# Mahdi-Si/VAE-TEB

Measured on AMD Instinct MI355X. Metric: train samples/sec + ELBO, 4096-pt windows, batch 256, 1/2/4/8 MI355X, higher is better.
Workload: dtype bf16 MFMA (decoder heads + conv blocks + ResidualMLP linears, LSTM recurrences f16 fwd / bf16 bwd), fp32 accumulation; fp32 LayerNorm / BatchNorm / LSTM state / front-end / optimizer

## Files before the change

### include/vaeteb.h

```cpp
#ifndef VAETEB_H
#define VAETEB_H

#include <stdint.h>

#ifdef __cplusplus
extern "C" {
#endif

#define VT_OK 0
#define VT_ERR_ARG (-1)
#define VT_ERR_LAYOUT (-2)
#define VT_ERR_HIP (-3)

#define VT_FFT_MAX_LDS 8192

const char* vt_last_error(void);
int vt_stream_fork(void* from, void* to);
int vt_stream_mark(void* stream, int* slot);
int vt_stream_wait_mark(void* stream, int slot);
int vt_abi_version(void);
int vt_arrive_reset(void* stream);
int vt_capture_info(void* stream, char* buf, int len);
int vt_set_h16_format(int fp16);
int vt_get_h16_format(void);
// ... 153 lines not shown
int vt_resmlp_bf16_fwd(int n_layers, const int* dims, const int* layer_ln, const int* layer_act, int skip, float eps,
                       const float* const* params, const float* x, int64_t rows, float* out, float* xhat, float* rstd,
                       void* stream);
int vt_resmlp_bf16_bwd(int n_layers, const int* dims, const int* layer_ln, const int* layer_act, int skip, float eps,
                       const float* const* params, const float* dout, const float* xhat, const float* rstd,
                       int64_t rows, float* dx, float* const* grads, int accumulate, float* ws, int64_t ws_floats,
                       void* stream);
int vt_resmlp_bf16_plan(int n_layers, const int* dims, const int* layer_ln, const int* layer_act, int skip, float eps,
                        const float* const* params, int64_t rows, int64_t* handle, void* stream);
int vt_resmlp_bf16_prep_batch(int n, const int64_t* handles, void* stream);
int vt_resmlp_bf16_fwd_prepped(int n_layers, const int* dims, const int* layer_ln, const int* layer_act, int skip,
                               float eps, const float* const* params, const float* x, int64_t rows, float* out,
                               float* xhat, float* rstd, void* stream);
int vt_resmlp_bf16_split_sizes(int n_layers, const int* dims, const int* layer_ln, const int* layer_act, int skip,
                               int64_t rows, int64_t* sizes);
int vt_resmlp_bf16_bwd_data(int n_layers, const int* dims, const int* layer_ln, const int* layer_act, int skip,
                            float eps, const float* const* params, const float* dout, const float* xhat,
                            const float* rstd, int64_t rows, float* dx, float* const* grads, int accumulate,
                            void* dz16, float* ws, int64_t ws_floats, void* stream);
int vt_resmlp_bf16_bwd_weight(int n_layers, const int* dims, const int* layer_ln, const int* layer_act, int skip,
                              float eps, const float* const* params, const float* xhat, const void* dz16,
                              int64_t rows, float* const* grads, int accumulate, float* ws, int64_t ws_floats,
                              void* stream);
int vt_resmlp_bf16_set_stamps(void* buf);

int vt_mfma_supported(int K, int N);
int vt_mfma_workspace_floats(int64_t R, int K, int N, int64_t* floats);
int vt_mfma_weight_shadow(const float* W, int N, int K, void* W16, void* W16t, void* stream);
int vt_mfma_linear_fwd(const float* X, int64_t R, int K, const void* W16, int N, const float* bias, float* Y,
                       float* ws, int64_t ws_floats, void* stream);
int vt_mfma_linear_bwd_data(const float* dY, int64_t R, int N, const void* W16t, int K, float* dX, int accumulate,
                            float* ws, int64_t ws_floats, void* stream);
int vt_mfma_linear_bwd_weight(const float* dY, int64_t R, int N, const float* X, int K, float* dW, float* db,
                              int accumulate, float* ws, int64_t ws_floats, void* stream);

int vt_conv1d_out_len(int L_in, int K, int mode, int up);
int vt_conv1d_fwd(const float* X, int B, int L_in, int Cin, const float* W, int Cout, int K, int mode, int up,
                  float* Y, void* stream);
int vt_conv1d_bwd_data(const float* dY, int B, int L_in, int Cin, const float* W, int Cout, int K, int mode, int up,
                       float* dX, int accumulate, float* gpad, void* stream);
int vt_conv1d_bwd_weight(const float* dY, const float* X, int B, int L_in, int Cin, int Cout, int K, int mode, int up,
                         float* dW, int accumulate, float* ws, int64_t ws_floats, void* stream);
int vt_conv1d_bn_workspace_floats(int B, int L_in, int Cin, int Cout, int K, int mode, int up, int64_t* floats);
int vt_conv1d_bn_fwd(const float* X, int B, int L_in, int Cin, const float* W, int Cout, int K, int mode, int up,
                     const float* gamma, const float* beta, int act, float eps, float momentum, float* conv_out,
                     float* Y, float* mean, float* rstd, float* run_mean, float* run_var, float* ws,
                     int64_t ws_floats, void* stream);
int vt_conv1d_bf16_shadow(const float* W, int Cout, int Cin, int K, void* w16, void* w16t, void* stream);
int vt_conv1d_bf16_shadow_batch(int n, const int64_t* W, const int* Cout, const int* Cin, const int* K,
                                const int64_t* w16, const int64_t* w16t, void* stream);
int vt_conv_bf16_set_staging(int mode);
int vt_conv_bf16_set_kernels(int flags);
int vt_conv1d_bn_fwd_bf16(const float* X, int B, int L_in, int Cin, const void* w16, int Cout, int K, int mode,
                          int up, const float* gamma, const float* beta, int act, float eps, float momentum,
                          float* conv_out, float* Y, float* mean, float* rstd, float* run_mean, float* run_var,
                          float* ws, int64_t ws_floats, void* stream);
int vt_conv1d_bn_fwd_bf16_in(const float* X, const float* in_mean, const float* in_rstd, const float* in_gamma,
                             const float* in_beta, int in_act, int B, int L_in, int Cin, const void* w16, int Cout,
                             int K, int mode, int up, const float* gamma, const float* beta, int act, float eps,
                             float momentum, float* conv_out, float* Y, float* mean, float* rstd, float* run_mean,
                             float* run_var, float* ws, int64_t ws_floats, void* stream);
int vt_conv1d_fwd_bf16(const float* X, int B, int L_in, int Cin, const void* w16, int Cout, int K, int mode, int up,
                       float* Y, void* stream);
int vt_conv1d_bwd_gpad_bf16(const float* dY, int B, int L_in, int Cin, const void* w16t, int Cout, int K, int mode,
                            int up, float* gpad, void* stream);
int vt_conv1d_bwd_weight_bf16(const float* dY, const float* X, int B, int L_in, int Cin, int Cout, int K, int mode,
                              int up, float* dW, int accumulate, float* ws, int64_t ws_floats, void* stream);
int vt_conv1d_bwd_gpad_bf16_bn(const float* dY, const float* Xc, const float* bnp, int act, int64_t M, int B,
                               int L_in, int Cin, const void* w16t, int Cout, int K, int mode, int up, float* gpad,
                               void* dxbn16, void* stream);
int vt_conv1d_bwd_dx_bf16_bn(const float* dY, const float* Xc, const float* bnp, int act, int64_t M, int B, int L_in,
                             int Cin, const void* w16t, int Cout, int K, int mode, int up, float* dX, float* edge,
                             void* dxbn16, void* stream);
int vt_conv1d_bwd_weight_bf16_dy16(const void* dY16, const float* X, int B, int L_in, int Cin, int Cout, int K,
                                   int mode, int up, float* dW, int accumulate, float* ws, int64_t ws_floats,
                                   void* stream);
int vt_conv1d_bwd_weight_bf16_dy16s(const void* dY16, int dys, const float* X, int B, int L_in, int Cin, int Cout,
                                    int K, int mode, int up, float* dW, int accumulate, float* ws, int64_t ws_floats,
                                    void* stream);
int vt_conv1d_bwd_weight_bf16_in(const float* dY, const void* dY16, int dys, const float* X, const float* in_mean,
                                 const float* in_rstd, const float* in_gamma, const float* in_beta, int in_act, int B,
                                 int L_in, int Cin, int Cout, int K, int mode, int up, float* dW, int accumulate,
                                 float* ws, int64_t ws_floats, void* stream);
int vt_batchnorm_bwd_x16(const float* dY, const float* Xc, const float* bnp, int act, int64_t M, int C, void* d16,
                         void* stream);
int vt_conv1d_bwd_dx16(const void* d16, int B, int L_in, int Cin, const void* w16t, int Cout, int K, int mode, int up,
                       float* dX, float* edge, void* stream);
int vt_conv1d_direct_fwd(const float* X, int B, int L_in, int Cin, const float* W, int Cout, int K, int mode, int up,
                         float* Y, void* stream);
int vt_conv1d_direct_bwd_gpad(const float* dY, int B, int L_in, int Cin, const float* W, int Cout, int K, int mode,
                              int up, float* gpad, void* stream);
int vt_conv1d_fold(const float* gpad, int B, int L_in, int Cin, int Cout, int K, int mode, int up, float* dX,
                   int accumulate, void* stream);
int vt_conv1d_direct_bwd_weight(const float* dY, const float* X, int B, int L_in, int Cin, int Cout, int K, int mode,
                                int up, float* dW, int accumulate, float* ws, int64_t ws_floats, void* stream);

int vt_layernorm_fwd(const float* x, int64_t R, int C, const float* gamma, const float* beta, int act, float eps,
                     float* y, float* xhat, float* rstd, void* stream);
int vt_layernorm_bwd(const float* dy, const float* xhat, const float* rstd, int64_t R, int C, const float* gamma,
                     const float* beta, int act, float* dx, float* dgamma, float* dbeta, int accumulate_params,
                     float* ws, int64_t ws_floats, void* stream);
int vt_batchnorm_fwd(const float* x, int64_t M, int C, const float* gamma, const float* beta, int act, float eps,
                     float momentum, float* y, float* mean, float* rstd, float* run_mean, float* run_var, float* ws,
                     int64_t ws_floats, void* stream);
int vt_batchnorm_bwd(const float* dy, const float* x, int64_t M, int C, const float* mean, const float* rstd,
                     const float* gamma, const float* beta, int act, float* dx, float* dgamma, float* dbeta,
                     int accumulate_params, float* ws, int64_t ws_floats, void* stream);
int vt_batchnorm_fwd_dropout(const float* x, int64_t M, int C, const float* gamma, const float* beta, int act,
                             float eps, float momentum, float* y, float* mean, float* rstd, float* run_mean,
                             float* run_var, int L, float p, int64_t seed, const void* seed_offset, float* ws,
                             int64_t ws_floats, void* stream);
int vt_batchnorm_bwd_dropout(const float* dy, const float* x, int64_t M, int C, const float* mean, const float* rstd,
                             const float* gamma, const float* beta, int act, int L, float p, int64_t seed,
                             const void* seed_offset, float* dx, float* dgamma, float* dbeta, int accumulate_params,
                             float* ws, int64_t ws_floats, void* stream);
int vt_batchnorm_bwd_coef(const float* dy, const float* x, int64_t M, int C, const float* mean, const float* rstd,
                          const float* gamma, const float* beta, int act, float* dgamma, float* dbeta,
                          int accumulate_params, float* bnp, float* ws, int64_t ws_floats, void* stream);
int vt_batchnorm_eval(const float* x, int64_t M, int C, const float* run_mean, const float* run_var, float eps,
                      const float* gamma, const float* beta, int act, float* y, void* stream);
int vt_syncbn_sums(const float* x, const float* dy, int64_t M, int C, int which, const float* mean,
                   const float* rstd, const float* gamma, const float* beta, int act, double* sums, float* ws,
                   int64_t ws_floats, void* stream);
int vt_syncbn_stats(const double* sums, int C, int which, float eps, float momentum, float* mean, float* rstd,
                    float* run_mean, float* run_var, float* dgamma, float* dbeta, int accumulate, void* stream);
int vt_batchnorm_apply(const float* x, int64_t M, int C, const float* mean, const float* rstd, const float* gamma,
                       const float* beta, int act, float* y, void* stream);
int vt_syncbn_bwd_dx(const float* dy, const float* x, int64_t M, int C, const float* mean, const float* rstd,
                     const float* gamma, const float* beta, int act, const double* sums, float* dx, float* ws,
                     void* stream);
int vt_act_fwd(const float* x, int64_t n, int act, float* y, void* stream);
int vt_act_bwd(const float* dy, const float* x, int64_t n, int act, float* dx, void* stream);

int vt_lstm_layer_fwd(const float* gin, const float* w_hh, const float* b_hh, int B, int S, int hidden, float* out_h,
                      float* out_hprev, float* out_c, float* gates, void* stream);
int vt_lstm_layer_bwd(const float* dh_out, const float* gates, const float* cst, const float* w_hh, int B, int S,
                      int hidden, float* dgates, void* stream);
int vt_lstm_layer_fwd_x(const float* x, int In, const float* w_ih, const float* b_ih, const float* w_hh,
                        const float* b_hh, int B, int S, int hidden, float* out_h, float* out_hprev, float* out_c,
                        float* gates, void* stream);
int vt_lstm_layer_bwd_x(const float* dh_out, const float* gates, const float* cst, const float* w_hh,
                        const float* w_ih, int In, int B, int S, int hidden, float* dgates, float* dx, void* stream);
int vt_lstm16_layer_fwd(const float* x, int In, const float* w_ih, const float* b_ih, const float* w_hh,
                        const float* b_hh, int B, int S, int hidden, float* out_h, float* out_hprev, float* out_c,
                        float* gates, void* stream);
int vt_lstm16_layer_bwd(const float* dh_out, const float* gates, const float* cst, const float* w_hh,
                        const float* w_ih, int In, int B, int S, int hidden, float* dgates, float* dx, void* stream);
int vt_lstm16_pair_fwd(const float* x, int In, const float* w_ih0, const float* b_ih0, const float* w_hh0,
                       const float* b_hh0, const float* w_ih1, const float* b_ih1, const float* w_hh1,
                       const float* b_hh1, int B, int seq, int hidden, float* h0, float* c0, float* gates0, float* h1,
                       float* c1, float* gates1, void* stream);
int vt_lstm16_pair_bwd(const float* dh_out, const float* gates1, const float* c1, const float* w_hh1,
                       const float* w_ih1, const float* gates0, const float* c0, const float* w_hh0,
                       const float* w_ih0, int In0, int B, int seq, int hidden, void* dgates1, void* dgates0,
                       float* dx, void* stream, int dg_bf16);
int vt_lstm16_quad_fwd(const float* x, int In, const float* const* params, int B, int seq, int hidden,
                       float* const* outs, void* stream);
int vt_lstm16_quad_bwd(const float* dh_out, const float* const* w, const float* const* gc, int In0, int B, int seq,
                       int hidden, void* const* dg, float* dmid, float* dx, void* stream, int dg_bf16);
int vt_lstm16_chain_errors(int* count, int reset);
int vt_lstm_layer_bwd_weight(const float* dgates, const float* x, int In, const float* hprev, int B, int S,
                             int hidden, float* dw_ih, float* dw_hh, float* db_ih, float* db_hh, int accumulate,
                             float* ws, int64_t ws_floats, void* stream);
int vt_lstm16_layer_bwd_weight(const float* dgates, const float* x, int In, const float* h, int B, int S,
                               int hidden, float* dw_ih, float* dw_hh, float* db_ih, float* db_hh, int accumulate,
                               float* ws, int64_t ws_floats, void* stream);
// ... 60 lines not shown
```

### vae-teb_amd/csrc/conv.h

```cpp
#pragma once
#include "bnbwd.h"
#include "common.h"

namespace vt {

struct Geo {
    int B, L_in, Cin, Cout, K, up, mode, L_up, pad, L_out;
};

__device__ __forceinline__ float up_lerp(float a, float b, float l1) {
#pragma clang fp contract(off)
    return (1.f - l1) * a + l1 * b;
}

template <bool IBN = false>
__device__ __forceinline__ float src_val(const float* __restrict__ xb, const Geo& g, int tp, int ci,
                                         const float* ip = nullptr, int cs = 0, int iact = 0) {
    int t = tp - g.pad;
    if (g.mode == 0) {
        if (t < 0 || t >= g.L_up) return 0.f;
    } else if (g.L_up <= g.pad) {
        t = t < 0 ? 0 : (t >= g.L_up ? g.L_up - 1 : t);
    } else {
        t = t < 0 ? -t : t;
        t = t >= g.L_up ? 2 * (g.L_up - 1) - t : t;
    }
    if (!g.up) {
        const float v = xb[(int64_t)t * g.Cin + ci];
        return IBN ? bn_relu_at(ip, cs, ci, v) : v;
    }
    float s = (t + 0.5f) * 0.5f - 0.5f;
    s = s < 0.f ? 0.f : s;
    const int i0 = (int)s;
    const int i1 = i0 + 1 < g.L_in ? i0 + 1 : g.L_in - 1;
    const float l1 = s - (float)i0;
    float a = xb[(int64_t)i0 * g.Cin + ci], b = xb[(int64_t)i1 * g.Cin + ci];
    if constexpr (IBN) {
        a = bn_relu_at(ip, cs, ci, a);
        b = bn_relu_at(ip, cs, ci, b);
    }
    return up_lerp(a, b, l1);
}


__device__ __forceinline__ bool src_row(const Geo& g, int tp, int& i0, int& i1, float& l1) {
    int t = tp - g.pad;
    if (g.mode == 0) {
        if (t < 0 || t >= g.L_up) return false;
    } else if (g.L_up <= g.pad) {
        t = t < 0 ? 0 : (t >= g.L_up ? g.L_up - 1 : t);
    } else {
        t = t < 0 ? -t : t;
        t = t >= g.L_up ? 2 * (g.L_up - 1) - t : t;
    }
    if (!g.up) {
        i0 = i1 = t;
        l1 = 0.f;
        return true;
    }
    float s = (t + 0.5f) * 0.5f - 0.5f;
    s = s < 0.f ? 0.f : s;
    i0 = (int)s;
    i1 = i0 + 1 < g.L_in ? i0 + 1 : g.L_in - 1;
    l1 = s - (float)i0;
    return true;
}

__device__ __forceinline__ void src_span(const Geo& g, int t0, int n, int& lo, int& hi) {
    const int ta = t0 - g.pad, tz = t0 + n - 1 - g.pad;
    int a = 0x7fffffff, z = -1;
    if (g.mode == 0) {
        a = ta > 0 ? ta : 0;
        z = tz < g.L_up - 1 ? tz : g.L_up - 1;
    } else if (g.L_up <= g.pad) {
        a = 0;
        z = g.L_up - 1;
    } else {
        if (tz >= 0 && ta <= g.L_up - 1) {
            a = ta > 0 ? ta : 0;
            z = tz < g.L_up - 1 ? tz : g.L_up - 1;
        }
        if (ta < 0) {
            const int l = -tz > 1 ? -tz : 1;
            a = l < a ? l : a;
            z = -ta > z ? -ta : z;
        }
        if (tz >= g.L_up) {
            const int l = 2 * (g.L_up - 1) - tz;
            const int h = 2 * (g.L_up - 1) - (ta > g.L_up ? ta : g.L_up);
            a = l < a ? l : a;
            z = h > z ? h : z;
        }
    }
    if (z < a) {
        lo = 0;
        hi = -1;
        return;
    }
    if (!g.up) {
        lo = a;
        hi = z;
        return;
    }
    float sa = (a + 0.5f) * 0.5f - 0.5f, sz = (z + 0.5f) * 0.5f - 0.5f;
    sa = sa < 0.f ? 0.f : sa;
    sz = sz < 0.f ? 0.f : sz;
    lo = (int)sa;
    hi = (int)sz + 1 < g.L_in ? (int)sz + 1 : g.L_in - 1;
}

template <int NC, bool IBN = false>
__device__ __forceinline__ void src_vec(const float* __restrict__ xb, const Geo& g, int tp, int cb, bool ok,
                                        float (&v)[NC], const float* ip = nullptr, int cs = 0, int iact = 0) {
    int i0 = 0, i1 = 0;
    float l1 = 0.f;
    const bool in = ok && src_row(g, tp, i0, i1, l1);
    const float* p0 = xb + (int64_t)(in ? i0 : 0) * g.Cin;
    const float* p1 = xb + (int64_t)(in ? i1 : 0) * g.Cin;
    float a[NC], b[NC];
#pragma unroll
    for (int j = 0; j < NC; ++j) {
        const int c = cb + j < g.Cin ? cb + j : g.Cin - 1;
        a[j] = p0[c];
        b[j] = g.up ? p1[c] : 0.f;
    }
    if constexpr (IBN) {
#pragma unroll
        for (int j = 0; j < NC; ++j) {
            a[j] = bn_relu_at(ip, cs, cb + j, a[j]);
            b[j] = g.up ? bn_relu_at(ip, cs, cb + j, b[j]) : 0.f;
        }
    }
#pragma unroll
    for (int j = 0; j < NC; ++j)
        v[j] = (in && cb + j < g.Cin) ? (g.up ? up_lerp(a[j], b[j], l1) : a[j]) : 0.f;
}

static inline Geo geo(int B, int L_in, int Cin, int Cout, int K, int mode, int up) {
    Geo g;
    g.B = B; g.L_in = L_in; g.Cin = Cin; g.Cout = Cout; g.K = K; g.mode = mode; g.up = up;
    g.L_up = L_in * (up ? 2 : 1);
    g.pad = mode == 0 ? K - 1 : (K - 1) / 2;
    g.L_out = mode == 0 ? g.L_up : g.L_up + 2 * g.pad - K + 1;
    return g;
}


static inline int cdiv(int a, int b) { return (a + b - 1) / b; }

int bn_stats_finalize_launch(const float* stats, int tiles_per_sample, int B, int TP, int Lo, int C, float eps,
                             float momentum, float* mean, float* rstd, float* run_mean, float* run_var,
                             hipStream_t st);
int sum_splits_launch(const float* part, int splits, int64_t n, float* out, int accumulate, hipStream_t st,
                      int pK = 0, int pCo = 0, int pCi = 0);
int cfw16_launch(const float* x, const Geo& g, const void* w16, float* y, int Lo, float* stats, hipStream_t st,
                 const BnIn* ibn = nullptr);
void fold_edges_launch(float* dx, const float* edge, int B, int L, int pad, int C, hipStream_t st);
int bn_apply_launch(const float* x, int64_t M, int C, const float* mean, const float* rstd, const float* gamma,
                    const float* beta, int act, float* y, hipStream_t st);

}
```

### vae-teb_amd/csrc/conv_bf16.hip

```cpp
#include <stdlib.h>

#include "conv.h"
#include "h16.h"

namespace vt {

int g_conv_kern = 11;

namespace {

constexpr int CB = 32;
constexpr int RS = 40;

template <int K, int NT>
struct BCfg {
    static constexpr int PM = NT <= 2 ? 4 : 2;
    static constexpr int TC = 16 * NT, TP = 64 * PM, WIN = TP + K - 1;
    static constexpr int XB = WIN * RS, WB = K * TC * RS;
    static constexpr int LDS_BYTES = (XB + WB) * 2 > 8 * TC * 4 ? (XB + WB) * 2 : 8 * TC * 4;
};

struct FoldOut {
    int pad, L;
    float* edge;
// ... 469 lines not shown
        case 10: return bf_k<10>(x, g, w16, cin32, y, Lo, stats, st, bn, fo, ibn);
        default: return bf_k<11>(x, g, w16, cin32, y, Lo, stats, st, bn, fo, ibn);
    }
}

__global__ void k_conv_fold_edges(float* __restrict__ dx, const float* __restrict__ edge, int L, int pad, int C) {
    const int i = blockIdx.x * blockDim.x + threadIdx.x;
    if (i >= 2 * pad * C) return;
    const int r = i / C, c = i - r * C, b = blockIdx.y;
    const int s = r < pad ? 1 + r : L - 1 - pad + (r - pad);
    if (s < 0 || s > L - 1 || (r < pad && s < 1) || (r >= pad && s >= 1 && s <= pad)) return;
    const float* eb = edge + (int64_t)b * 2 * pad * C + c;
    float* o = dx + ((int64_t)b * L + s) * C + c;
    float v = *o;
    if (s >= 1 && s <= pad) v += eb[(pad - s) * C];
    const int tr = pad + 2 * (L - 1) - s;
    if (s <= L - 2 && tr < L + 2 * pad && tr >= pad + L) v += eb[(tr - L) * C];
    *o = v;
}

constexpr int KMAXB = 11;

}

void fold_edges_launch(float* dx, const float* edge, int B, int L, int pad, int C, hipStream_t st) {
    hipLaunchKernelGGL(k_conv_fold_edges, dim3((unsigned)((2 * pad * C + 255) / 256), (unsigned)B), dim3(256), 0, st,
                       dx, edge, L, pad, C);
}
}

using namespace vt;

extern "C" {

int vt_conv_bf16_set_staging(int mode) {
    VT_CHECK_ARG(mode >= 0 && mode <= 2, "vt_conv_bf16_set_staging: mode %d not in 0..2", mode);
    g_conv_cl = mode;
    return VT_OK;
}

int vt_conv_bf16_set_kernels(int flags) {
    VT_CHECK_ARG(flags >= 0 && flags <= 15, "vt_conv_bf16_set_kernels: flags %d not in 0..15", flags);
    g_conv_kern = flags;
    return VT_OK;
}

int vt_conv1d_bf16_shadow(const float* W, int Cout, int Cin, int K, void* w16, void* w16t, void* stream) {
    VT_CHECK_ARG(Cout > 0 && Cin > 0 && K > 0 && K <= KMAXB, "vt_conv1d_bf16_shadow: shape");
    const int cin32 = cdiv(Cin, 32) * 32, cout32 = cdiv(Cout, 32) * 32;
    const int64_t n = (int64_t)Cout * K * cin32 + (int64_t)Cin * K * cout32;
    VT_H16(hipLaunchKernelGGL(k_conv_shadow<H>, dim3((unsigned)((n + 255) / 256)), dim3(256), 0, S(stream), W, Cout,
                              Cin, K, cin32, cout32, (H*)w16, (H*)w16t));
    VT_LAUNCH_CHECK("vt_conv1d_bf16_shadow");
    return VT_OK;
}

int vt_conv1d_bf16_shadow_batch(int n, const int64_t* W, const int* Cout, const int* Cin, const int* K,
                                const int64_t* w16, const int64_t* w16t, void* stream) {
    VT_CHECK_ARG(n >= 0 && n <= CSB_MAX, "vt_conv1d_bf16_shadow_batch: %d weights (at most %d)", n, CSB_MAX);
    if (n == 0) return VT_OK;
    ConvShadowBatch cb{};
    cb.n = n;
    cb.prefix[0] = 0;
    for (int h = 0; h < n; ++h) {
        VT_CHECK_ARG(W[h] && w16[h] && w16t[h] && Cout[h] > 0 && Cin[h] > 0 && K[h] > 0 && K[h] <= KMAXB,
                     "vt_conv1d_bf16_shadow_batch: weight %d", h);
        cb.W[h] = reinterpret_cast<const float*>(W[h]);
        cb.Cout[h] = Cout[h];
        cb.Cin[h] = Cin[h];
        cb.K[h] = K[h];
        cb.w16[h] = reinterpret_cast<void*>(w16[h]);
        cb.w16t[h] = reinterpret_cast<void*>(w16t[h]);
        const int64_t e = (int64_t)Cout[h] * K[h] * (cdiv(Cin[h], 32) * 32) + (int64_t)Cin[h] * K[h] * (cdiv(Cout[h], 32) * 32);
        cb.prefix[h + 1] = cb.prefix[h] + (int)((e + 255) / 256);
    }
    VT_H16(hipLaunchKernelGGL(k_conv_shadow_batch<H>, dim3((unsigned)cb.prefix[n]), dim3(256), 0, S(stream), cb));
    VT_LAUNCH_CHECK("vt_conv1d_bf16_shadow_batch");
    return VT_OK;
}

static int bn_fwd_bf16(const float* X, int B, int L_in, int Cin, const void* w16, int Cout, int K, int mode, int up,
                       const float* gamma, const float* beta, int act, float eps, float momentum, float* conv_out,
                       float* Y, float* mean, float* rstd, float* run_mean, float* run_var, float* ws,
                       int64_t ws_floats, hipStream_t st, const BnIn* ibn, const char* who) {
    VT_CHECK_ARG(B > 0 && L_in > 0 && Cin > 0 && Cout > 0 && K > 0 && K <= KMAXB && (mode == 0 || mode == 1),
                 "%s: shape (K <= %d)", who, KMAXB);
    Geo g = geo(B, L_in, Cin, Cout, K, mode, up);
    const int cin32 = cdiv(Cin, 32) * 32;
    const int TP = bf_launch(nullptr, g, nullptr, cin32, nullptr, g.L_out, nullptr, nullptr);
    const int tps = cdiv(g.L_out, TP);
    VT_CHECK_ARG(ws && ws_floats >= (int64_t)B * tps * 2 * Cout, "%s: workspace too small", who);
    if (bf_launch(X, g, w16, cin32, conv_out, g.L_out, ws, st, nullptr, FoldOut{-1, 0, nullptr}, ibn) < 0) return VT_ERR_ARG;
    bn_stats_finalize_launch(ws, tps, B, TP, g.L_out, Cout, eps, momentum, mean, rstd, run_mean, run_var, st);
    if (Y) bn_apply_launch(conv_out, (int64_t)B * g.L_out, Cout, mean, rstd, gamma, beta, act, Y, st);
    VT_LAUNCH_CHECK(who);
    return VT_OK;
}

int vt_conv1d_bn_fwd_bf16(const float* X, int B, int L_in, int Cin, const void* w16, int Cout, int K, int mode,
                          int up, const float* gamma, const float* beta, int act, float eps, float momentum,
                          float* conv_out, float* Y, float* mean, float* rstd, float* run_mean, float* run_var,
                          float* ws, int64_t ws_floats, void* stream) {
    return bn_fwd_bf16(X, B, L_in, Cin, w16, Cout, K, mode, up, gamma, beta, act, eps, momentum, conv_out, Y, mean,
                       rstd, run_mean, run_var, ws, ws_floats, S(stream), nullptr, "vt_conv1d_bn_fwd_bf16");
}

int vt_conv1d_bn_fwd_bf16_in(const float* X, const float* in_mean, const float* in_rstd, const float* in_gamma,
                             const float* in_beta, int in_act, int B, int L_in, int Cin, const void* w16, int Cout,
                             int K, int mode, int up, const float* gamma, const float* beta, int act, float eps,
                             float momentum, float* conv_out, float* Y, float* mean, float* rstd, float* run_mean,
                             float* run_var, float* ws, int64_t ws_floats, void* stream) {
    VT_CHECK_ARG(in_mean && in_rstd && in_gamma && in_beta && in_act == 1,
                 "vt_conv1d_bn_fwd_bf16_in: input BatchNorm parameters (ReLU blocks only)");
    const BnIn bi{in_mean, in_rstd, in_gamma, in_beta, in_act};
    return bn_fwd_bf16(X, B, L_in, Cin, w16, Cout, K, mode, up, gamma, beta, act, eps, momentum, conv_out, Y, mean,
                       rstd, run_mean, run_var, ws, ws_floats, S(stream), &bi, "vt_conv1d_bn_fwd_bf16_in");
}

int vt_conv1d_fwd_bf16(const float* X, int B, int L_in, int Cin, const void* w16, int Cout, int K, int mode, int up,
                       float* Y, void* stream) {
    VT_CHECK_ARG(B > 0 && L_in > 0 && Cin > 0 && Cout > 0 && K > 0 && K <= KMAXB && (mode == 0 || mode == 1),
                 "vt_conv1d_fwd_bf16: shape (K <= %d)", KMAXB);
    Geo g = geo(B, L_in, Cin, Cout, K, mode, up);
    if (bf_launch(X, g, w16, cdiv(Cin, 32) * 32, Y, g.L_out, nullptr, S(stream)) < 0) return VT_ERR_ARG;
    VT_LAUNCH_CHECK("vt_conv1d_fwd_bf16");
    return VT_OK;
}

static int bwd_gpad(const float* dY, int B, int L_in, int Cin, const void* w16t, int Cout, int K, int mode, int up,
                    float* gpad, hipStream_t st, const BnB* bn, const char* who,
                    FoldOut fo = FoldOut{-1, 0, nullptr}) {
    VT_CHECK_ARG(B > 0 && L_in > 0 && Cin > 0 && Cout > 0 && K > 0 && K <= KMAXB, "%s: shape", who);
    Geo f = geo(B, L_in, Cin, Cout, K, mode, up);
    Geo g = geo(B, f.L_out, Cout, Cin, K, 0, 0);
    if (bf_launch(dY, g, w16t, cdiv(Cout, 32) * 32, gpad, f.L_out + K - 1, nullptr, st, bn, fo) < 0) return VT_ERR_ARG;
    VT_LAUNCH_CHECK(who);
    return VT_OK;
}

int vt_conv1d_bwd_gpad_bf16(const float* dY, int B, int L_in, int Cin, const void* w16t, int Cout, int K, int mode,
                            int up, float* gpad, void* stream) {
    return bwd_gpad(dY, B, L_in, Cin, w16t, Cout, K, mode, up, gpad, S(stream), nullptr, "vt_conv1d_bwd_gpad_bf16");
}

int vt_conv1d_bwd_gpad_bf16_bn(const float* dY, const float* Xc, const float* bnp, int act, int64_t M, int B,
                               int L_in, int Cin, const void* w16t, int Cout, int K, int mode, int up, float* gpad,
                               void* dxbn16, void* stream) {
    VT_CHECK_ARG(Xc && bnp && act >= 0 && act <= 3 && M > 0, "vt_conv1d_bwd_gpad_bf16_bn: BatchNorm arguments");
    const BnB bn{Xc, bnp, act, 1.f / (float)M, dxbn16};
    return bwd_gpad(dY, B, L_in, Cin, w16t, Cout, K, mode, up, gpad, S(stream), &bn, "vt_conv1d_bwd_gpad_bf16_bn");
}

int vt_conv1d_bwd_dx_bf16_bn(const float* dY, const float* Xc, const float* bnp, int act, int64_t M, int B, int L_in,
                             int Cin, const void* w16t, int Cout, int K, int mode, int up, float* dX, float* edge,
                             void* dxbn16, void* stream) {
    VT_CHECK_ARG(Xc && bnp && act >= 0 && act <= 3 && M > 0, "vt_conv1d_bwd_dx_bf16_bn: BatchNorm arguments");
    const Geo f = geo(B, L_in, Cin, Cout, K, mode, up);
    VT_CHECK_ARG(!up && (mode == 0 || f.L_up > f.pad) && (mode == 0 || f.pad == 0 || edge),
                 "vt_conv1d_bwd_dx_bf16_bn: geometry (no upsample, reflect needs L > pad and an edge buffer)");
    const BnB bn{Xc, bnp, act, 1.f / (float)M, dxbn16};
    const FoldOut fo{f.pad, L_in, mode == 0 ? nullptr : edge};
    const int rc = bwd_gpad(dY, B, L_in, Cin, w16t, Cout, K, mode, up, dX, S(stream), &bn,
                            "vt_conv1d_bwd_dx_bf16_bn", fo);
    if (rc) return rc;
    if (mode == 1 && f.pad > 0) {
        VT_CHECK_ARG(B <= 65535, "vt_conv1d_bwd_dx_bf16_bn: batch");
        fold_edges_launch(dX, edge, B, L_in, f.pad, Cin, S(stream));
        VT_LAUNCH_CHECK("vt_conv1d_bwd_dx_bf16_bn");
    }
    return VT_OK;
}

}
```

### vae-teb_amd/csrc/conv_dw16.hip

```cpp
#include "conv.h"
#include "h16.h"

namespace vt {

extern int g_conv_kern;

namespace {

constexpr int KMAXB = 11;

typedef short v4i16 __attribute__((ext_vector_type(4)));
constexpr int DWR = 64;
constexpr int KMAXB_DW = 11;

template <typename H>
__device__ __forceinline__ hv8<H> tr_frag(const H* img, int row0, int col0, int stride) {
    const int lane = threadIdx.x & 63, g = lane >> 4, q = (lane >> 2) & 3, p = lane & 3;
    const H* a0 = img + (row0 + 8 * g + q) * stride + col0 + 4 * p;
    const v4i16 lo = __builtin_amdgcn_ds_read_tr16_b64_v4i16((__attribute__((address_space(3))) v4i16*)a0);
    const v4i16 hi = __builtin_amdgcn_ds_read_tr16_b64_v4i16(
        (__attribute__((address_space(3))) v4i16*)(a0 + 4 * stride));
    typedef short v8i16 __attribute__((ext_vector_type(8)));
    const v8i16 r = __builtin_shufflevector(lo, hi, 0, 1, 2, 3, 4, 5, 6, 7);
    return __builtin_bit_cast(hv8<H>, r);
// ... 63 lines not shown
                    if (i < nd) *(v4s*)(ds + t * dstride + c) = v[u];
                }
            }
        } else {
            for (int i0 = tid; i0 < nd; i0 += 64 * NWV * UR) {
                float v[UR][4];
#pragma unroll
                for (int u = 0; u < UR; ++u) {
                    const int i = i0 + 64 * NWV * u;
                    const int t = i / (cout16 / 4), c = 4 * (i - t * (cout16 / 4));
                    const bool ok = i < nd && t < n;
#pragma unroll
                    for (int j = 0; j < 4; ++j) {
                        const int cc = c + j < g.Cout ? c + j : g.Cout - 1;
                        v[u][j] = dyb[(int64_t)(ok ? t : 0) * g.Cout + cc];
                        v[u][j] = (ok && c + j < g.Cout) ? v[u][j] : 0.f;
                    }
                }
#pragma unroll
                for (int u = 0; u < UR; ++u) {
                    const int i = i0 + 64 * NWV * u;
                    const int t = i / (cout16 / 4), c = 4 * (i - t * (cout16 / 4));
                    if (i < nd)
#pragma unroll
                        for (int j = 0; j < 4; ++j) ds[t * dstride + c + j] = (H)v[u][j];
                }
            }
        }
        for (int i0 = tid; i0 < nx; i0 += 64 * NWV * UR) {
            float v[UR][4];
#pragma unroll
            for (int u = 0; u < UR; ++u) {
                const int i = i0 + 64 * NWV * u;
                const int t = i / (cin16 / 4), c = 4 * (i - t * (cin16 / 4));
                src_vec<4, IBN>(xb, g, t0 + t, c, i < nx && t < n + K - 1, v[u], ip, ics, bi.act);
            }
#pragma unroll
            for (int u = 0; u < UR; ++u) {
                const int i = i0 + 64 * NWV * u;
                const int t = i / (cin16 / 4), c = 4 * (i - t * (cin16 / 4));
                if (i < nx)
#pragma unroll
                    for (int j = 0; j < 4; ++j) xs[t * xstride + c + j] = (H)v[u][j];
            }
        }
        __syncthreads();
#pragma unroll
        for (int s = 0; s < DWR / 32; ++s) {
            if (!act[0]) break;
#pragma unroll
            for (int j = 0; j < PPW; ++j) {
                const hv8<H> a = tr_frag<H>(ds, 32 * s, 16 * mt[j], dstride);
#pragma unroll
                for (int k = 0; k < K; ++k) {
                    const hv8<H> bb = tr_frag<H>(xs, 32 * s + k, 16 * nt[j], xstride);
                    acc[j][k] = mfma16(a, bb, acc[j][k]);
                }
            }
        }
        __syncthreads();
        r += n;
    }
    const int64_t slot = blockIdx.y;
#pragma unroll
    for (int j = 0; j < PPW; ++j) {
        if (!act[j]) continue;
        const int ci = 16 * nt[j] + lr;
        if (ci >= g.Cin) continue;
#pragma unroll
        for (int rr = 0; rr < 4; ++rr) {
            const int co = 16 * mt[j] + 4 * lc + rr;
            if (co >= g.Cout) continue;
            float* pp = part + ((slot * g.Cout + co) * g.Cin + ci) * K;
#pragma unroll
            for (int k = 0; k < K; ++k) pp[k] = acc[j][k][rr];
        }
    }
}

constexpr int CDW_UD = 4;
constexpr int CDW_UF = 8;
constexpr int CDW_UF_WIDE = 12;

template <int K, int PPW, int NWV, int CR = DWR, bool IBN = false, typename H = __bf16>
__global__ __launch_bounds__(64 * NWV) void k_cdw16(const H* __restrict__ dyb16, int dys,
                                                   const float* __restrict__ x, Geo g, int64_t rows_per_split,
                                                   int NTc, int npairs, int dstride, int xstride,
                                                   float* __restrict__ part, int64_t total, BnIn bi, int ipo) {
    constexpr int NT = 64 * NWV;
    constexpr int UD = CR == DWR ? CDW_UD * 256 / NT : CR * 4 / NT;
    constexpr int UF = CR == DWR ? CDW_UF * 256 / NT : CDW_UF_WIDE * 256 / NT;
    extern __shared__ __attribute__((aligned(16))) char lb_raw[];
    H* const lb = reinterpret_cast<H*>(lb_raw);
    H* ds = lb;
    H* xs = lb + CR * dstride;
    float* F = reinterpret_cast<float*>(lb + CR * dstride + (CR + KMAXB_DW + 8) * xstride);
    const int tid = threadIdx.x, lane = tid & 63, wv = tid >> 6;
    int mt[PPW], nt[PPW];
    bool act[PPW];
#pragma unroll
    for (int j = 0; j < PPW; ++j) {
        const int p = blockIdx.x * (NWV * PPW) + wv + NWV * j;
        act[j] = p < npairs;
        mt[j] = act[j] ? p / NTc : 0;
        nt[j] = act[j] ? p - mt[j] * NTc : 0;
    }
    const int64_t rows = (int64_t)g.B * g.L_out;
    const int64_t r0 = (int64_t)blockIdx.y * rows_per_split;
    const int64_t r1 = r0 + rows_per_split < rows ? r0 + rows_per_split : rows;
    f32x4 acc[PPW][K];
#pragma unroll
    for (int j = 0; j < PPW; ++j)
#pragma unroll
        for (int k = 0; k < K; ++k) acc[j][k] = f32x4{0.f, 0.f, 0.f, 0.f};
    const int cout16 = (g.Cout + 15) / 16 * 16, cin16 = (g.Cin + 15) / 16 * 16;
    const int dsegs = cout16 / 8;
    float* ip = reinterpret_cast<float*>(reinterpret_cast<char*>(lb) + ipo);
    if constexpr (IBN) stage_bn_in(bi, g.Cin, ip, cin16);
    hv8<H> dv[UD];
    float4 fv[UF];
    struct Chunk {
        int b, t0, n, lo, hi, off, nv;
    };
    auto load = [&](int64_t r, Chunk& c) {
        c.b = (int)(r / g.L_out);
        c.t0 = (int)(r - (int64_t)c.b * g.L_out);
        c.n = g.L_out - c.t0 < CR ? g.L_out - c.t0 : CR;
        if (r + c.n > r1) c.n = (int)(r1 - r);
        const H* db = dyb16 + ((int64_t)c.b * g.L_out + c.t0) * dys;
#pragma unroll
        for (int u = 0; u < UD; ++u) {
            const int i = tid + NT * u;
            const int t = i / dsegs, sg = i - t * dsegs;
            const bool ok = i < CR * dsegs && t < c.n && 8 * sg < dys;
            dv[u] = *(const hv8<H>*)(db + (int64_t)(ok ? t : 0) * dys + (ok ? 8 * sg : 0));
            if (!ok) {
#pragma unroll
                for (int j = 0; j < 8; ++j) dv[u][j] = (H)0.f;
            }
        }
        src_span(g, c.t0, c.n + K - 1, c.lo, c.hi);
        const int64_t f0 = ((int64_t)c.b * g.L_in + c.lo) * g.Cin;
        const int64_t fa = f0 & ~(int64_t)3;
        c.off = (int)(f0 - fa);
        const int nf = c.hi >= c.lo ? (int)(((int64_t)c.b * g.L_in + c.hi + 1) * g.Cin - fa) : 0;
        const int nv = (nf + 3) >> 2;
        c.nv = nv;
#pragma unroll
        for (int u = 0; u < UF; ++u) {
            const int i = tid + NT * u;
            const int64_t e = fa + 4 * (int64_t)i;
            if (i < nv && e + 3 < total) {
                fv[u] = *reinterpret_cast<const float4*>(x + e);
            } else {
                fv[u].x = i < nv && e < total ? x[e] : 0.f;
                fv[u].y = i < nv && e + 1 < total ? x[e + 1] : 0.f;
                fv[u].z = i < nv && e + 2 < total ? x[e + 2] : 0.f;
                fv[u].w = 0.f;
            }
        }
    };
    Chunk cur;
    if (r0 < r1) load(r0, cur);
    for (int64_t r = r0; r < r1;) {
#pragma unroll
        for (int u = 0; u < UD; ++u) {
            const int i = tid + NT * u;
            if (i < CR * dsegs) {
                const int t = i / dsegs, sg = i - t * dsegs;
                *(hv8<H>*)(ds + t * dstride + 8 * sg) = dv[u];
            }
        }
#pragma unroll
        for (int u = 0; u < UF; ++u)
            if (tid + NT * u < cur.nv) reinterpret_cast<float4*>(F)[tid + NT * u] = fv[u];
        __syncthreads();
        {
            const int osegs = cin16 / 8;
            for (int i = tid; i < (CR + K - 1) * osegs; i += NT) {
                const int t = i / osegs, o = i - t * osegs;
                const int tp = cur.t0 + t, cb = 8 * o;
                int i0 = 0, i1 = 0;
                float l1 = 0.f;
                const bool in = t < cur.n + K - 1 && src_row(g, tp, i0, i1, l1);
                const float* p0 = F + cur.off + (in ? i0 - cur.lo : 0) * g.Cin;
                const float* p1 = F + cur.off + (in ? i1 - cur.lo : 0) * g.Cin;
                hv8<H> v;
#pragma unroll
                for (int j = 0; j < 8; ++j) {
                    const int c = cb + j < g.Cin ? cb + j : g.Cin - 1;
                    float a = p0[c];
                    float q = g.up ? p1[c] : 0.f;
                    if constexpr (IBN) {
                        a = bn_relu_at(ip, cin16, cb + j, a);
                        q = g.up ? bn_relu_at(ip, cin16, cb + j, q) : 0.f;
                    }
                    v[j] = (H)((in && cb + j < g.Cin) ? (g.up ? up_lerp(a, q, l1) : a) : 0.f);
                }
                *(hv8<H>*)(xs + t * xstride + cb) = v;
            }
        }
        __syncthreads();
        const int64_t rn = r + cur.n;
        Chunk nxt = cur;
        if (rn < r1) load(rn, nxt);
#pragma unroll
        for (int s = 0; s < CR / 32; ++s) {
            if (!act[0]) break;
#pragma unroll
            for (int j = 0; j < PPW; ++j) {
                const hv8<H> a = tr_frag<H>(ds, 32 * s, 16 * mt[j], dstride);
#pragma unroll
                for (int k = 0; k < K; ++k) {
                    const hv8<H> bb = tr_frag<H>(xs, 32 * s + k, 16 * nt[j], xstride);
                    acc[j][k] = mfma16(a, bb, acc[j][k]);
                }
            }
        }
        __syncthreads();
        cur = nxt;
        r = rn;
    }
    const int lr = lane & 15, lc = lane >> 4;
    const int64_t slot = blockIdx.y;
#pragma unroll
    for (int j = 0; j < PPW; ++j) {
        if (!act[j]) continue;
        const int ci = 16 * nt[j] + lr;
        if (ci >= g.Cin) continue;
#pragma unroll
        for (int rr = 0; rr < 4; ++rr) {
            const int co = 16 * mt[j] + 4 * lc + rr;
            if (co >= g.Cout) continue;
            float* pp = part + ((slot * g.Cout + co) * g.Cin + ci) * K;
#pragma unroll
            for (int k = 0; k < K; ++k) pp[k] = acc[j][k][rr];
        }
    }
}

}
}

using namespace vt;

extern "C" {

static int bwd_weight(const float* dY, const float* X, int B, int L_in, int Cin, int Cout, int K, int mode, int up,
                      float* dW, int accumulate, float* ws, int64_t ws_floats, hipStream_t st, const void* dy16,
                      int dys = 0, const BnIn* ibn = nullptr) {
    VT_CHECK_ARG(B > 0 && L_in > 0 && K > 0 && K <= KMAXB && Cin > 0 && Cout > 0 && Cin <= 128 && Cout <= 128,
                 "vt_conv1d_bwd_weight_bf16: shape (K <= %d, channels <= 128)", KMAXB);
    Geo g = geo(B, L_in, Cin, Cout, K, mode, up);
    const int NTc = cdiv(Cin, 16), npairs = cdiv(Cout, 16) * NTc;
    const int ppw_max = K <= 3 ? 6 : (K <= 5 ? 4 : (K <= 7 ? 3 : 2));
    const int ppw = cdiv(npairs, 4) < ppw_max ? cdiv(npairs, 4) : ppw_max;
    const int need = cdiv(npairs, ppw);
    const int nwv = !dy16 || need <= 4 ? 4 : 8;
    const int bx = cdiv(npairs, nwv * ppw);
    const int64_t rows = (int64_t)B * g.L_out;
    const int64_t nout = (int64_t)Cout * Cin * K;
    constexpr int CONVDW_WG = 8192;
    int64_t splits = CONVDW_WG / (nwv * bx);
    if (splits > 1024) splits = 1024;
    if (splits * nout > (int64_t)8 << 20) splits = ((int64_t)8 << 20) / nout;
    if (splits > rows / (4 * DWR)) splits = rows / (4 * DWR);
    if (splits < 1) splits = 1;
    if (splits * nout > ws_floats) splits = ws_floats / nout;
    VT_CHECK_ARG(splits >= 1, "vt_conv1d_bwd_weight_bf16: workspace too small");
    int64_t rps = (rows + splits - 1) / splits;
    splits = (rows + rps - 1) / rps;
    const int dstride = 16 * cdiv(Cout, 16) + 8, xstride = 16 * cdiv(Cin, 16) + 8;
    const size_t lds = (size_t)(DWR * dstride + (DWR + KMAXB + 8) * xstride) * 2;
    if (dys == 0) dys = (Cout + 7) & ~7;
    dim3 grid(bx, (unsigned)splits);
    const int f_rows = (up ? (DWR + K - 1) / 2 + 3 : DWR + K - 1);
    const int64_t f_floats = (int64_t)f_rows * Cin + 8;
    const bool flat_ok = dy16 && ((uintptr_t)X & 15) == 0 && ((uintptr_t)dy16 & 15) == 0 && dys % 8 == 0;
    const bool flat = flat_ok && (g_conv_kern & 2) && (K >= 7 || (g_conv_kern & 4)) &&
                      f_floats <= (int64_t)4 * CDW_UF * 256 && 16 * cdiv(Cout, 16) <= 8 * CDW_UD * 32;
    const size_t lds_flat = lds + (size_t)f_floats * 4 + 64;
    const int64_t total_x = (int64_t)B * L_in * Cin;
    const int fw_rows = up ? (256 + K - 1) / 2 + 3 : 256 + K - 1;
    const int64_t fw_floats = (int64_t)fw_rows * Cin + 8;
    const bool wide = flat_ok && (g_conv_kern & 8) && cdiv(Cout, 16) <= 2 &&
                      fw_floats <= (int64_t)4 * CDW_UF_WIDE * 256 && rps >= 256;
    const size_t lds_wide = (size_t)(256 * dstride + (256 + KMAXB + 8) * xstride) * 2 + (size_t)fw_floats * 4 + 64;
    const BnIn bi = ibn ? *ibn : BnIn{};
    const int ib = ibn ? 16 * (16 * cdiv(Cin, 16)) : 0;
    const int ipo_w = ((int)lds_wide + 15) & ~15, ipo_f = ((int)lds_flat + 15) & ~15, ipo_d = ((int)lds + 15) & ~15;
#define VT_DWB_ONE(IB, HT)                                                                                      \
    if (wide && nwv == 8)                                                                                       \
        hipLaunchKernelGGL((k_cdw16<KK, PP, 8, 256, IB, HT>), grid, dim3(512), ipo_w + ib, st, (const HT*)dy16,   \
                           dys, X, g, rps, NTc, npairs, dstride, xstride, ws, total_x, bi, ipo_w);             \
    else if (wide)                                                                                              \
        hipLaunchKernelGGL((k_cdw16<KK, PP, 4, 256, IB, HT>), grid, dim3(256), ipo_w + ib, st, (const HT*)dy16,   \
                           dys, X, g, rps, NTc, npairs, dstride, xstride, ws, total_x, bi, ipo_w);             \
    else if (flat && nwv == 8)                                                                                  \
        hipLaunchKernelGGL((k_cdw16<KK, PP, 8, DWR, IB, HT>), grid, dim3(512), ipo_f + ib, st, (const HT*)dy16,   \
                           dys, X, g, rps, NTc, npairs, dstride, xstride, ws, total_x, bi, ipo_f);             \
    else if (flat)                                                                                              \
        hipLaunchKernelGGL((k_cdw16<KK, PP, 4, DWR, IB, HT>), grid, dim3(256), ipo_f + ib, st, (const HT*)dy16,   \
                           dys, X, g, rps, NTc, npairs, dstride, xstride, ws, total_x, bi, ipo_f);             \
    else if (dy16 && nwv == 8)                                                                                  \
        hipLaunchKernelGGL((k_conv_dw_bf16<KK, PP, true, 8, IB, HT>), grid, dim3(512), ipo_d + ib, st, dY, X, g,  \
                           rps, NTc, npairs, dstride, xstride, ws, (const HT*)dy16, dys, bi, ipo_d);           \
    else if (dy16)                                                                                              \
        hipLaunchKernelGGL((k_conv_dw_bf16<KK, PP, true, 4, IB, HT>), grid, dim3(256), ipo_d + ib, st, dY, X, g,  \
                           rps, NTc, npairs, dstride, xstride, ws, (const HT*)dy16, dys, bi, ipo_d);           \
    else if (!IB)                                                                                               \
        hipLaunchKernelGGL((k_conv_dw_bf16<KK, PP, false, 4, false, HT>), grid, dim3(256), ipo_d, st, dY, X, g,   \
                           rps, NTc, npairs, dstride, xstride, ws, (const HT*)nullptr, 0, bi, ipo_d);
    const bool f16 = h16_format() != 0;
    VT_CHECK_ARG(!(f16 && ibn), "vt_conv1d_bwd_weight_bf16_in: the conv-stack fold has no fp16 form");
#define VT_DWB(KK_, PP_)                    \
    if (K == KK_ && ppw == PP_) {           \
        constexpr int KK = KK_, PP = PP_;   \
        if (f16) {                          \
            VT_DWB_ONE(false, _Float16)     \
        } else if (ibn) {                   \
            VT_DWB_ONE(true, __bf16)        \
        } else {                            \
            VT_DWB_ONE(false, __bf16)       \
        }                                   \
    }
#define VT_DWB6(KK) VT_DWB(KK, 1) VT_DWB(KK, 2) VT_DWB(KK, 3) VT_DWB(KK, 4) VT_DWB(KK, 5) VT_DWB(KK, 6)
#define VT_DWB4(KK) VT_DWB(KK, 1) VT_DWB(KK, 2) VT_DWB(KK, 3) VT_DWB(KK, 4)
#define VT_DWB3(KK) VT_DWB(KK, 1) VT_DWB(KK, 2) VT_DWB(KK, 3)
#define VT_DWB2(KK) VT_DWB(KK, 1) VT_DWB(KK, 2)
    VT_DWB6(1) VT_DWB6(2) VT_DWB6(3) VT_DWB4(4) VT_DWB4(5) VT_DWB3(6) VT_DWB3(7)
    VT_DWB2(8) VT_DWB2(9) VT_DWB2(10) VT_DWB2(11)
#undef VT_DWB6
#undef VT_DWB4
#undef VT_DWB3
#undef VT_DWB2
#undef VT_DWB
#undef VT_DWB_ONE
    const int rc = sum_splits_launch(ws, (int)splits, nout, dW, accumulate, st);
    if (rc) return rc;
    VT_LAUNCH_CHECK("vt_conv1d_bwd_weight_bf16");
    return VT_OK;
}

int vt_conv1d_bwd_weight_bf16(const float* dY, const float* X, int B, int L_in, int Cin, int Cout, int K, int mode,
                              int up, float* dW, int accumulate, float* ws, int64_t ws_floats, void* stream) {
    return bwd_weight(dY, X, B, L_in, Cin, Cout, K, mode, up, dW, accumulate, ws, ws_floats, S(stream), nullptr);
}

int vt_conv1d_bwd_weight_bf16_dy16(const void* dY16, const float* X, int B, int L_in, int Cin, int Cout, int K,
                                   int mode, int up, float* dW, int accumulate, float* ws, int64_t ws_floats,
                                   void* stream) {
    VT_CHECK_ARG(dY16 != nullptr, "vt_conv1d_bwd_weight_bf16_dy16: null dY16");
    return bwd_weight(nullptr, X, B, L_in, Cin, Cout, K, mode, up, dW, accumulate, ws, ws_floats, S(stream), dY16);
}

int vt_conv1d_bwd_weight_bf16_dy16s(const void* dY16, int dys, const float* X, int B, int L_in, int Cin, int Cout,
                                    int K, int mode, int up, float* dW, int accumulate, float* ws, int64_t ws_floats,
                                    void* stream) {
    VT_CHECK_ARG(dY16 != nullptr && dys >= ((Cout + 7) & ~7) && dys % 8 == 0,
                 "vt_conv1d_bwd_weight_bf16_dy16s: null dY16 or row stride %d (a multiple of 8 >= ceil8(Cout))", dys);
    return bwd_weight(nullptr, X, B, L_in, Cin, Cout, K, mode, up, dW, accumulate, ws, ws_floats, S(stream),
                      dY16, dys);
}

int vt_conv1d_bwd_weight_bf16_in(const float* dY, const void* dY16, int dys, const float* X, const float* in_mean,
                                 const float* in_rstd, const float* in_gamma, const float* in_beta, int in_act, int B,
                                 int L_in, int Cin, int Cout, int K, int mode, int up, float* dW, int accumulate,
                                 float* ws, int64_t ws_floats, void* stream) {
    VT_CHECK_ARG(in_mean && in_rstd && in_gamma && in_beta && in_act == 1,
                 "vt_conv1d_bwd_weight_bf16_in: input BatchNorm parameters (ReLU blocks only)");
    VT_CHECK_ARG(dY16 && dys >= ((Cout + 7) & ~7) && dys % 8 == 0,
                 "vt_conv1d_bwd_weight_bf16_in: bf16 dY16 (row stride %d) required", dys);
    (void)dY;
    const BnIn bi{in_mean, in_rstd, in_gamma, in_beta, in_act};
    return bwd_weight(dY, X, B, L_in, Cin, Cout, K, mode, up, dW, accumulate, ws, ws_floats, S(stream),
                      dY16, dY16 ? dys : 0, &bi);
}

}
```

### vae-teb_amd/csrc/conv_fwd16.hip

```cpp
#include "conv.h"
#include "h16.h"

namespace vt {

namespace {


constexpr int RS = 40;

template <int K, int NT>
struct FCfg {
    static constexpr int PM = NT <= 2 ? 4 : 2;
    static constexpr int TC = 16 * NT, TP = 64 * PM, WIN = TP + K - 1;
    static constexpr int NWI = (K * TC * 4 + 255) / 256;
    static constexpr int WBYTES = K * TC * RS * 2;
};

template <int K, int NT, bool IBN = false, typename H = __bf16>
__global__ __launch_bounds__(256) void k_cfw16(const float* __restrict__ x, Geo g, int nch,
                                               const H* __restrict__ w16, float* __restrict__ y, int Lo,
                                               float* __restrict__ stats, int64_t total, BnIn bi, int ipo) {
    using C = FCfg<K, NT>;
    constexpr int PM = C::PM, TC = C::TC, TP = C::TP, WIN = C::WIN;
    extern __shared__ __attribute__((aligned(16))) char lb_raw[];
    H* const lb = reinterpret_cast<H*>(lb_raw);
    const int cin32 = 32 * nch;
    H* xs = lb;
    char* rest = reinterpret_cast<char*>(lb + nch * WIN * RS);
    float* F = reinterpret_cast<float*>(rest);
    H* ws = reinterpret_cast<H*>(rest);
    const int tid = threadIdx.x, lane = tid & 63, wv = tid >> 6, lr = lane & 15, lc = lane >> 4;
    const int t0 = blockIdx.x * TP, co0 = blockIdx.y * TC, b = blockIdx.z;
    hv8<H> wt[C::NWI];
    auto load_taps = [&](int c0) {
#pragma unroll
        for (int it = 0; it < C::NWI; ++it) {
            const int i = tid + 256 * it;
            const int ic = i < K * TC * 4 ? i : K * TC * 4 - 1;
            const int oct = ic & 3, r = ic >> 2, k = r / TC, co = r - k * TC;
            const int coc = co0 + co < g.Cout ? co0 + co : g.Cout - 1;
            wt[it] = *(const hv8<H>*)(w16 + ((int64_t)coc * K + k) * cin32 + c0 + 8 * oct);
        }
    };
    load_taps(0);
    float* ip = reinterpret_cast<float*>(reinterpret_cast<char*>(lb) + ipo);
    if constexpr (IBN) stage_bn_in(bi, g.Cin, ip, cin32);
    int lo, hi;
    src_span(g, t0, WIN < Lo + K - 1 - t0 ? WIN : Lo + K - 1 - t0, lo, hi);
    const int64_t f0 = ((int64_t)b * g.L_in + lo) * g.Cin;
    const int64_t fa = f0 & ~(int64_t)3;
    const int nf = hi >= lo ? (int)(((int64_t)b * g.L_in + hi + 1) * g.Cin - fa) : 0;
    const int nv = (nf + 3) >> 2;
    {
        constexpr int U = 12;
        for (int i0 = tid; i0 < nv; i0 += 256 * U) {
            float4 v[U];
#pragma unroll
            for (int u = 0; u < U; ++u) {
                const int i = i0 + 256 * u;
                const int64_t e = fa + 4 * (int64_t)i;
                if (i < nv && e + 3 < total) {
                    v[u] = *reinterpret_cast<const float4*>(x + e);
                } else {
                    v[u].x = i < nv && e < total ? x[e] : 0.f;
                    v[u].y = i < nv && e + 1 < total ? x[e + 1] : 0.f;
                    v[u].z = i < nv && e + 2 < total ? x[e + 2] : 0.f;
                    v[u].w = 0.f;
                }
            }
#pragma unroll
            for (int u = 0; u < U; ++u) {
                const int i = i0 + 256 * u;
                if (i < nv) reinterpret_cast<float4*>(F)[i] = v[u];
            }
        }
    }
    __syncthreads();
    {
        const int segs = 4 * nch;
        const int off = (int)(f0 - fa);
        for (int i = tid; i < WIN * segs; i += 256) {
            const int r = i / segs, s = i - r * segs;
            const int tp = t0 + r, cb = 8 * s;
            int i0 = 0, i1 = 0;
            float l1 = 0.f;
            const bool in = tp < Lo + K - 1 && src_row(g, tp, i0, i1, l1);
            const float* p0 = F + off + (in ? i0 - lo : 0) * g.Cin;
            const float* p1 = F + off + (in ? i1 - lo : 0) * g.Cin;
            hv8<H> v;
#pragma unroll
            for (int j = 0; j < 8; ++j) {
                const int c = cb + j < g.Cin ? cb + j : g.Cin - 1;
                float a = p0[c];
                float q = g.up ? p1[c] : 0.f;
                if constexpr (IBN) {
                    a = bn_relu_at(ip, cin32, cb + j, a);
                    q = g.up ? bn_relu_at(ip, cin32, cb + j, q) : 0.f;
                }
                v[j] = (H)((in && cb + j < g.Cin) ? (g.up ? up_lerp(a, q, l1) : a) : 0.f);
            }
            *(hv8<H>*)(xs + ((s >> 2) * WIN + r) * RS + 8 * (s & 3)) = v;
        }
    }
    __syncthreads();
    auto store_taps = [&]() {
#pragma unroll
        for (int it = 0; it < C::NWI; ++it) {
            const int i = tid + 256 * it;
            if (i >= K * TC * 4) continue;
            const int oct = i & 3, r = i >> 2, k = r / TC, co = r - k * TC;
            hv8<H> v = wt[it];
            if (co0 + co >= g.Cout) {
#pragma unroll
                for (int j = 0; j < 8; ++j) v[j] = (H)0.f;
            }
            *(hv8<H>*)(ws + (k * TC + co) * RS + 8 * oct) = v;
        }
    };
    store_taps();
    __syncthreads();
    f32x4 acc[PM][NT];
#pragma unroll
    for (int m = 0; m < PM; ++m)
#pragma unroll
        for (int n = 0; n < NT; ++n) acc[m][n] = f32x4{0.f, 0.f, 0.f, 0.f};
    for (int ch = 0; ch < nch; ++ch) {
        const bool more = ch + 1 < nch;
        if (more) load_taps(32 * (ch + 1));
        const H* xq = xs + (ch * WIN + PM * 16 * wv + lr) * RS + 8 * lc;
        const H* wq = ws + lr * RS + 8 * lc;
#pragma unroll
        for (int k = 0; k < K; ++k) {
            hv8<H> af[PM], bf[NT];
#pragma unroll
            for (int m = 0; m < PM; ++m) af[m] = *(const hv8<H>*)(xq + (16 * m + k) * RS);
#pragma unroll
            for (int n = 0; n < NT; ++n) bf[n] = *(const hv8<H>*)(wq + (k * TC + 16 * n) * RS);
#pragma unroll
            for (int m = 0; m < PM; ++m)
#pragma unroll
                for (int n = 0; n < NT; ++n)
                    acc[m][n] = mfma16(af[m], bf[n], acc[m][n]);
        }
        __syncthreads();
        if (more) {
            store_taps();
            __syncthreads();
        }
    }
#pragma unroll
    for (int m = 0; m < PM; ++m)
#pragma unroll
        for (int r = 0; r < 4; ++r) {
            const int t = t0 + PM * 16 * wv + 16 * m + 4 * lc + r;
            if (t >= Lo) continue;
            float* yr = y + ((int64_t)b * Lo + t) * g.Cout;
#pragma unroll
            for (int n = 0; n < NT; ++n) {
                const int co = co0 + 16 * n + lr;
                if (co < g.Cout) yr[co] = acc[m][n][r];
            }
        }
    if (stats) {
        float* red1 = reinterpret_cast<float*>(lb);
        float* red2 = red1 + 4 * TC;
        const int nrow = Lo - t0 < TP ? Lo - t0 : TP;
        float cs[NT];
#pragma unroll
        for (int n = 0; n < NT; ++n) {
            float a = 0.f;
#pragma unroll
            for (int m = 0; m < PM; ++m)
#pragma unroll
                for (int r = 0; r < 4; ++r)
                    if (t0 + PM * 16 * wv + 16 * m + 4 * lc + r < Lo) a += acc[m][n][r];
            a += __shfl_xor(a, 16);
            a += __shfl_xor(a, 32);
            cs[n] = a;
        }
        if (lc == 0)
#pragma unroll
            for (int n = 0; n < NT; ++n) red1[wv * TC + 16 * n + lr] = cs[n];
        __syncthreads();
#pragma unroll
        for (int n = 0; n < NT; ++n) {
            const int c = 16 * n + lr;
            const float mu = (((red1[c] + red1[TC + c]) + red1[2 * TC + c]) + red1[3 * TC + c]) / (float)nrow;
            float q = 0.f;
#pragma unroll
            for (int m = 0; m < PM; ++m)
#pragma unroll
                for (int r = 0; r < 4; ++r)
                    if (t0 + PM * 16 * wv + 16 * m + 4 * lc + r < Lo) {
                        const float dlt = acc[m][n][r] - mu;
                        q += dlt * dlt;
                    }
            q += __shfl_xor(q, 16);
            q += __shfl_xor(q, 32);
            if (lc == 0) red2[wv * TC + c] = q;
        }
        __syncthreads();
        if (tid < TC && co0 + tid < g.Cout) {
            const int64_t tile = (int64_t)b * gridDim.x + blockIdx.x;
            const int64_t ntile = (int64_t)gridDim.z * gridDim.x;
            float* sp = stats + (int64_t)(co0 + tid) * ntile + tile;
            sp[0] = ((red1[tid] + red1[TC + tid]) + red1[2 * TC + tid]) + red1[3 * TC + tid];
            sp[(int64_t)g.Cout * ntile] = ((red2[tid] + red2[TC + tid]) + red2[2 * TC + tid]) + red2[3 * TC + tid];
        }
    }
}

template <int K, int NT>
int cfw_nt(const float* x, const Geo& g, const void* w16, float* y, int Lo, float* stats, hipStream_t st,
           const BnIn* ibn) {
    using C = FCfg<K, NT>;
    const int nch = cdiv(g.Cin, 32);
    const int src_rows = g.up ? C::WIN / 2 + 3 : C::WIN;
    const int fbytes = (src_rows * g.Cin + 8) * 4;
    const int rest = fbytes > C::WBYTES ? fbytes : C::WBYTES;
    int lds = nch * C::WIN * RS * 2 + rest;
    if (lds < 8 * C::TC * 4) lds = 8 * C::TC * 4;
    const int ipo = (lds + 15) & ~15;
    if (ibn) lds = ipo + 4 * 32 * nch * 4;
    if (lds > 160 * 1024) return VT_ERR_ARG;
    dim3 grid(cdiv(Lo, C::TP), cdiv(g.Cout, C::TC), g.B);
    const int64_t total = (int64_t)g.B * g.L_in * g.Cin;
    const BnIn bi = ibn ? *ibn : BnIn{};
    if (h16_format()) {
        if (ibn) return VT_ERR_ARG;
        hipLaunchKernelGGL((k_cfw16<K, NT, false, _Float16>), grid, dim3(256), lds, st, x, g, nch,
                           (const _Float16*)w16, y, Lo, stats, total, bi, ipo);
    } else if (ibn)
        hipLaunchKernelGGL((k_cfw16<K, NT, true, __bf16>), grid, dim3(256), lds, st, x, g, nch, (const __bf16*)w16, y, Lo, stats,
                           total, bi, ipo);
    else
        hipLaunchKernelGGL((k_cfw16<K, NT, false, __bf16>), grid, dim3(256), lds, st, x, g, nch, (const __bf16*)w16, y, Lo, stats,
                           total, bi, ipo);
    return C::TP;
}

template <int K>
int cfw_k(const float* x, const Geo& g, const void* w16, float* y, int Lo, float* stats, hipStream_t st,
          const BnIn* ibn) {
    switch (cdiv(g.Cout, 16) < 6 ? cdiv(g.Cout, 16) : 6) {
        case 1: return cfw_nt<K, 1>(x, g, w16, y, Lo, stats, st, ibn);
        case 2: return cfw_nt<K, 2>(x, g, w16, y, Lo, stats, st, ibn);
        case 3: return cfw_nt<K, 3>(x, g, w16, y, Lo, stats, st, ibn);
        case 4: return cfw_nt<K, 4>(x, g, w16, y, Lo, stats, st, ibn);
        case 5: return cfw_nt<K, 5>(x, g, w16, y, Lo, stats, st, ibn);
        default: return cfw_nt<K, 6>(x, g, w16, y, Lo, stats, st, ibn);
    }
}

}

int cfw16_launch(const float* x, const Geo& g, const void* w16, float* y, int Lo, float* stats, hipStream_t st,
                 const BnIn* ibn) {
    switch (g.K) {
        case 1: return cfw_k<1>(x, g, w16, y, Lo, stats, st, ibn);
        case 2: return cfw_k<2>(x, g, w16, y, Lo, stats, st, ibn);
        case 3: return cfw_k<3>(x, g, w16, y, Lo, stats, st, ibn);
        case 4: return cfw_k<4>(x, g, w16, y, Lo, stats, st, ibn);
        case 5: return cfw_k<5>(x, g, w16, y, Lo, stats, st, ibn);
        case 6: return cfw_k<6>(x, g, w16, y, Lo, stats, st, ibn);
        case 7: return cfw_k<7>(x, g, w16, y, Lo, stats, st, ibn);
        case 8: return cfw_k<8>(x, g, w16, y, Lo, stats, st, ibn);
        case 9: return cfw_k<9>(x, g, w16, y, Lo, stats, st, ibn);
        case 10: return cfw_k<10>(x, g, w16, y, Lo, stats, st, ibn);
        default: return cfw_k<11>(x, g, w16, y, Lo, stats, st, ibn);
    }
}

}
```

### vae-teb_amd/csrc/norm.hip

```cpp
#include <math.h>

#include "bnbwd.h"
#include "common.h"
#include "dropout.h"

namespace vt {

enum Act { ACT_NONE = 0, ACT_RELU = 1, ACT_GELU = 2, ACT_TANH = 3 };

__device__ __forceinline__ float act_f(float z, int act) {
    switch (act) {
        case ACT_RELU: return z > 0.f ? z : 0.f;
        case ACT_GELU: return 0.5f * z * (1.f + erff(z * 0.70710678118654752f));
        case ACT_TANH: return tanhf(z);
        default: return z;
    }
}
__device__ __forceinline__ float act_d(float z, int act) {
    switch (act) {
        case ACT_RELU: return z > 0.f ? 1.f : 0.f;
        case ACT_GELU: {
            const float cdf = 0.5f * (1.f + erff(z * 0.70710678118654752f));
            const float pdf = 0.39894228040143268f * expf(-0.5f * z * z);
            return cdf + z * pdf;
        }
        case ACT_TANH: {
            const float t = tanhf(z);
            return 1.f - t * t;
        }
        default: return 1.f;
    }
}

static constexpr int NT = 256;

__global__ __launch_bounds__(NT) void k_ln_fwd(const float* __restrict__ x, int64_t R, int C,
                                               const float* __restrict__ gamma, const float* __restrict__ beta,
                                               int act, float eps, float* __restrict__ y, float* __restrict__ xhat,
                                               float* __restrict__ rstd_out) {
    const int lane = threadIdx.x & 63;
    const int64_t row = (int64_t)blockIdx.x * (NT / 64) + (threadIdx.x >> 6);
    if (row >= R) return;
    const float* xr = x + row * C;
    float s = 0.f;
    for (int c = lane; c < C; c += 64) s += xr[c];
    const float mean = wave_sum(s) / (float)C;
    float v = 0.f;
    for (int c = lane; c < C; c += 64) {
        const float d = xr[c] - mean;
        v += d * d;
    }
    const float rstd = rsqrtf(wave_sum(v) / (float)C + eps);
    float* yr = y + row * C;
    float* hr = xhat ? xhat + row * C : nullptr;
    for (int c = lane; c < C; c += 64) {
        const float h = (xr[c] - mean) * rstd;
        if (hr) hr[c] = h;
        yr[c] = act_f(h * gamma[c] + beta[c], act);
    }
    if (lane == 0 && rstd_out) rstd_out[row] = rstd;
}

template <int V4>
__global__ __launch_bounds__(NT) void k_ln_fwd_wide(const float* __restrict__ x, int C, const float* __restrict__ gamma,
                                                    const float* __restrict__ beta, int act, float eps,
                                                    float* __restrict__ y, float* __restrict__ xhat,
                                                    float* __restrict__ rstd_out) {
    __shared__ float red[16];
    const int64_t row = blockIdx.x;
    const float4* xr = reinterpret_cast<const float4*>(x + row * C);
    const int C4 = C >> 2;
    float4 v[V4];
    float s = 0.f;
#pragma unroll
    for (int j = 0; j < V4; ++j) {
        const int c4 = threadIdx.x + NT * j;
        v[j] = c4 < C4 ? xr[c4] : make_float4(0.f, 0.f, 0.f, 0.f);
        s += (v[j].x + v[j].y) + (v[j].z + v[j].w);
    }
    const float mean = block_sum(s, red) / (float)C;
    float q = 0.f;
#pragma unroll
    for (int j = 0; j < V4; ++j) {
        const int c4 = threadIdx.x + NT * j;
        if (c4 < C4) {
            const float a = v[j].x - mean, b = v[j].y - mean, c = v[j].z - mean, d = v[j].w - mean;
            q += (a * a + b * b) + (c * c + d * d);
// ... 408 lines not shown
    }
    __syncthreads();
    if (tid < C) bn_fin_channel(tid, C, fin[tid], fin[C + tid], f);
}

__global__ void k_bn_apply(const float* __restrict__ x, int64_t M, int C, const float* __restrict__ mean,
                           const float* __restrict__ rstd, const float* __restrict__ gamma,
                           const float* __restrict__ beta, int act, float* __restrict__ y) {
    const int64_t i = (int64_t)blockIdx.x * blockDim.x + threadIdx.x;
    if (i >= M * C) return;
    const int c = (int)(i % C);
    y[i] = bn_fwd_val(x[i], mean[c], rstd[c], gamma[c], beta[c], act);
}

__global__ void k_bn_eval(const float* __restrict__ x, int64_t M, int C, const float* __restrict__ run_mean,
                          const float* __restrict__ run_var, float eps, const float* __restrict__ gamma,
                          const float* __restrict__ beta, int act, float* __restrict__ y) {
    const int64_t i = (int64_t)blockIdx.x * blockDim.x + threadIdx.x;
    if (i >= M * C) return;
    const int c = (int)(i % C);
    y[i] = act_f((x[i] - run_mean[c]) * (1.f / sqrtf(run_var[c] + eps)) * gamma[c] + beta[c], act);
}

__global__ void k_act_fwd(const float* __restrict__ x, int64_t n, int act, float* __restrict__ y) {
    const int64_t i = (int64_t)blockIdx.x * blockDim.x + threadIdx.x;
    if (i < n) y[i] = act_f(x[i], act);
}
__global__ void k_act_bwd(const float* __restrict__ dy, const float* __restrict__ x, int64_t n, int act,
                          float* __restrict__ dx) {
    const int64_t i = (int64_t)blockIdx.x * blockDim.x + threadIdx.x;
    if (i < n) dx[i] = dy[i] * act_d(x[i], act);
}

static constexpr int BNV_C = 1024;
static constexpr int BNV_V = 4;

__device__ __forceinline__ int wrapc(int c, int C) { return c >= C ? c - C : c; }

__device__ __forceinline__ void chan4(int c, int C, int (&ce)[4]) {
    if (C >= 4) {
        ce[0] = c;
        ce[1] = wrapc(c + 1, C);
        ce[2] = wrapc(ce[1] + 1, C);
        ce[3] = wrapc(ce[2] + 1, C);
    } else {
#pragma unroll
        for (int e = 0; e < 4; ++e) ce[e] = (c + e) % C;
    }
}

template <int ACT>
__global__ __launch_bounds__(NT) void k_bn_apply4(const float* __restrict__ x, int64_t n, int C,
                                                  const float* __restrict__ mean, const float* __restrict__ rstd,
                                                  const float* __restrict__ gamma, const float* __restrict__ beta,
                                                  float* __restrict__ y) {
    __shared__ float4 p[BNV_C];
    for (int c = threadIdx.x; c < C; c += NT) p[c] = make_float4(mean[c], rstd[c], gamma[c], beta[c]);
    __syncthreads();
    const int64_t base = (int64_t)blockIdx.x * (NT * 4 * BNV_V);
    const int step = (NT * 4) % C;
    int c = (int)((base + 4 * threadIdx.x) % C);
#pragma unroll
    for (int v = 0; v < BNV_V; ++v, c = wrapc(c + step, C)) {
        const int64_t j = base + 4 * (threadIdx.x + NT * v);
        if (j >= n) break;
        int ce[4];
        chan4(c, C, ce);
        if (j + 4 <= n) {
            const float4 xv = *(const float4*)(x + j);
            const float xs[4] = {xv.x, xv.y, xv.z, xv.w};
            float o[4];
#pragma unroll
            for (int e = 0; e < 4; ++e) {
                const float4 q = p[ce[e]];
                o[e] = bn_fwd_val(xs[e], q.x, q.y, q.z, q.w, ACT);
            }
            *(float4*)(y + j) = make_float4(o[0], o[1], o[2], o[3]);
        } else {
            for (int e = 0; e < (int)(n - j); ++e) {
                const float4 q = p[ce[e]];
                y[j + e] = bn_fwd_val(x[j + e], q.x, q.y, q.z, q.w, ACT);
            }
        }
    }
}

struct DropArg {
    int L;
    float p;
    uint64_t seed;
    const uint64_t* soff;
};
__device__ __forceinline__ float dmask(const DropArg& d, uint64_t seed, uint32_t th, float sc, int64_t i, int C,
                                       int ch, float g) {
    const uint64_t m = d.L > 0 ? (uint64_t)((i / ((int64_t)d.L * C)) * C + ch) : (uint64_t)i;
    return mix_hash(seed, m) >= th ? g * sc : 0.f;
}

template <int ACT>
__global__ __launch_bounds__(NT) void k_bn_apply4d(const float* __restrict__ x, int64_t n, int C,
                                                   const float* __restrict__ mean, const float* __restrict__ rstd,
                                                   const float* __restrict__ gamma, const float* __restrict__ beta,
                                                   float* __restrict__ y, int L, float p, uint64_t seed,
                                                   const uint64_t* __restrict__ soff) {
    __shared__ float4 q4[BNV_C];
    for (int c = threadIdx.x; c < C; c += NT) q4[c] = make_float4(mean[c], rstd[c], gamma[c], beta[c]);
    __syncthreads();
    seed = eff_seed(seed, soff);
    const uint32_t th = drop_threshold(p);
    const float sc = 1.f / (1.f - p);
    const int64_t LC = (int64_t)L * C;
    auto drop = [&](int64_t i, int ch, float v) {
        const uint64_t m = L > 0 ? (uint64_t)((i / LC) * C + ch) : (uint64_t)i;
        return mix_hash(seed, m) >= th ? v * sc : 0.f;
    };
    const int64_t base = (int64_t)blockIdx.x * (NT * 4 * BNV_V);
    const int step = (NT * 4) % C;
    int c = (int)((base + 4 * threadIdx.x) % C);
#pragma unroll
    for (int v = 0; v < BNV_V; ++v, c = wrapc(c + step, C)) {
        const int64_t j = base + 4 * (threadIdx.x + NT * v);
        if (j >= n) break;
        int ce[4];
        chan4(c, C, ce);
        if (j + 4 <= n) {
            const float4 xv = *(const float4*)(x + j);
            const float xs[4] = {xv.x, xv.y, xv.z, xv.w};
            float o[4];
#pragma unroll
            for (int e = 0; e < 4; ++e) {
                const float4 q = q4[ce[e]];
                o[e] = drop(j + e, ce[e], bn_fwd_val(xs[e], q.x, q.y, q.z, q.w, ACT));
            }
            *(float4*)(y + j) = make_float4(o[0], o[1], o[2], o[3]);
        } else {
            for (int e = 0; e < (int)(n - j); ++e) {
                const float4 q = q4[ce[e]];
                y[j + e] = drop(j + e, ce[e], bn_fwd_val(x[j + e], q.x, q.y, q.z, q.w, ACT));
            }
        }
    }
}

template <int ACT, bool DROP = false>
__global__ __launch_bounds__(NT) void k_bn_dx4(const float* __restrict__ dy, const float* __restrict__ x, int64_t n,
                                               int64_t M, int C, const float* __restrict__ mean,
                                               const float* __restrict__ rstd, const float* __restrict__ gamma,
                                               const float* __restrict__ beta, const float* __restrict__ dgamma,
                                               const float* __restrict__ dbeta, float* __restrict__ dx,
                                               DropArg dr = DropArg{}) {
    __shared__ float p[6][BNV_C];
    for (int c = threadIdx.x; c < C; c += NT) {
        p[0][c] = mean[c];
        p[1][c] = rstd[c];
        p[2][c] = gamma[c];
        p[3][c] = beta[c];
        p[4][c] = dgamma[c];
        p[5][c] = dbeta[c];
    }
    __syncthreads();
    const float inv = 1.f / (float)M;
    const int64_t base = (int64_t)blockIdx.x * (NT * 4 * BNV_V);
    const int step = (NT * 4) % C;
    int c = (int)((base + 4 * threadIdx.x) % C);
    auto one = [&](float xe, float dye, int cc) { return bn_bwd_val(dye, xe, &p[0][0], BNV_C, cc, ACT, inv); };
    const uint64_t dseed = DROP ? eff_seed(dr.seed, dr.soff) : 0;
// ... 237 lines not shown

static void col_partial_fin(int kind, const float* x, const float* dy, int64_t M, int C, int64_t rpb, int blocks,
                            const float* mean, const float* rstd, const float* gamma, const float* beta, int act,
                            float* ws, hipStream_t st, BnFin f, const DropArg* dr = nullptr) {
    if (C <= 128) {
        const int ng = (blocks + BN_GB - 1) / BN_GB;
        f.gpart = reinterpret_cast<double*>(ws + (((int64_t)2 * C * blocks + 1) & ~(int64_t)1));
        f.slot0 = arrive_slots((unsigned)ng + 1, st);
        col_partial_vec(kind, x, dy, M, C, rpb, blocks, mean, rstd, gamma, beta, act, ws, st, f, dr);
    } else {
        col_partial_vec(kind, x, dy, M, C, rpb, blocks, mean, rstd, gamma, beta, act, ws, st, no_fin(), dr);
        hipLaunchKernelGGL(k_bn_finalize, dim3(C), dim3(NT), 0, st, ws, blocks, C, f);
    }
}

static inline unsigned blocks_for(int64_t n, int t = 256) { return (unsigned)((n + t - 1) / t); }

__global__ __launch_bounds__(NT) void k_sbn_sums(const float* __restrict__ part, int blocks, int C, int64_t M,
                                                 double* __restrict__ sums) {
    __shared__ double r0[NT], r1[NT];
    const int c = blockIdx.x;
    double a0 = 0.0, a1 = 0.0;
    const float* p0 = part + (int64_t)c * blocks;
    const float* p1 = part + (int64_t)(C + c) * blocks;
    for (int b = threadIdx.x; b < blocks; b += NT) {
        a0 += (double)p0[b];
        a1 += (double)p1[b];
    }
    r0[threadIdx.x] = a0;
    r1[threadIdx.x] = a1;
    __syncthreads();
    for (int o = NT / 2; o > 0; o >>= 1) {
        if (threadIdx.x < o) {
            r0[threadIdx.x] += r0[threadIdx.x + o];
            r1[threadIdx.x] += r1[threadIdx.x + o];
        }
        __syncthreads();
    }
    if (threadIdx.x == 0) {
        sums[c] = r0[0];
        sums[C + c] = r1[0];
        if (c == 0) sums[2 * C] = (double)M;
    }
}

__global__ void k_sbn_stats(const double* __restrict__ sums, int C, int which, float eps, float momentum,
                            float* __restrict__ mean, float* __restrict__ rstd, float* __restrict__ run_mean,
                            float* __restrict__ run_var, float* __restrict__ dgamma, float* __restrict__ dbeta,
                            int accumulate) {
    const int c = blockIdx.x * blockDim.x + threadIdx.x;
    if (c >= C) return;
    const double M = sums[2 * C];
    if (which == 0) {
        mean[c] = (float)(sums[c] / M);
    } else if (which == 1) {
        const double var = sums[c] / M;
        rstd[c] = (float)(1.0 / sqrt(var + (double)eps));
        if (run_mean) {
            const double unb = M > 1 ? var * M / (M - 1) : var;
            run_mean[c] = (float)((1.0 - momentum) * run_mean[c] + momentum * mean[c]);
            run_var[c] = (float)((1.0 - momentum) * run_var[c] + momentum * unb);
        }
    } else {
        dbeta[c] = accumulate ? dbeta[c] + (float)sums[c] : (float)sums[c];
        dgamma[c] = accumulate ? dgamma[c] + (float)sums[C + c] : (float)sums[C + c];
    }
}

__global__ void k_sbn_dsum(const double* __restrict__ sums, int C, float* __restrict__ dg, float* __restrict__ db) {
    const int c = blockIdx.x * blockDim.x + threadIdx.x;
    if (c >= C) return;
    const double M = sums[2 * C];
    db[c] = (float)(sums[c] / M);
    dg[c] = (float)(sums[C + c] / M);
}

int bn_apply_launch(const float* x, int64_t M, int C, const float* mean, const float* rstd, const float* gamma,
                    const float* beta, int act, float* y, hipStream_t st) {
    if (C <= BNV_C)
        bn_apply_vec(x, M, C, mean, rstd, gamma, beta, act, y, st);
    else
        hipLaunchKernelGGL(k_bn_apply, dim3(blocks_for(M * C)), dim3(256), 0, st, x, M, C, mean, rstd, gamma, beta,
                           act, y);
    return VT_OK;
}

}

using namespace vt;

extern "C" {

int vt_layernorm_fwd(const float* x, int64_t R, int C, const float* gamma, const float* beta, int act, float eps,
                     float* y, float* xhat, float* rstd, void* stream) {
    VT_CHECK_ARG(R > 0 && C > 0 && act >= 0 && act <= 3, "vt_layernorm_fwd: shape/act");
    if (C <= 256) {
        const dim3 grid((unsigned)((R + NT / 16 - 1) / (NT / 16)));
        hipStream_t st = S(stream);
        if (C <= 32)
            hipLaunchKernelGGL(k_ln_fwd16<2>, grid, dim3(NT), 0, st, x, R, C, gamma, beta, act, eps, y, xhat, rstd);
        else if (C <= 64)
            hipLaunchKernelGGL(k_ln_fwd16<4>, grid, dim3(NT), 0, st, x, R, C, gamma, beta, act, eps, y, xhat, rstd);
        else if (C <= 128)
            hipLaunchKernelGGL(k_ln_fwd16<8>, grid, dim3(NT), 0, st, x, R, C, gamma, beta, act, eps, y, xhat, rstd);
        else
            hipLaunchKernelGGL(k_ln_fwd16<16>, grid, dim3(NT), 0, st, x, R, C, gamma, beta, act, eps, y, xhat, rstd);
        VT_LAUNCH_CHECK("vt_layernorm_fwd");
        return VT_OK;
    }
    if (C >= 1024 && C % 4 == 0 && C <= 4 * 4 * NT && ((uintptr_t)x | (uintptr_t)y | (uintptr_t)gamma |
                                                       (uintptr_t)beta | (uintptr_t)xhat) % 16 == 0) {
        const int v4 = (C / 4 + NT - 1) / NT;
        hipStream_t st = S(stream);
#define VT_LNW(V)                                                                                              \
    if (v4 == V) hipLaunchKernelGGL(k_ln_fwd_wide<V>, dim3((unsigned)R), dim3(NT), 0, st, x, C, gamma, beta, act, eps, \
                                    y, xhat, rstd);
        VT_LNW(1) VT_LNW(2) VT_LNW(3) VT_LNW(4)
#undef VT_LNW
        VT_LAUNCH_CHECK("vt_layernorm_fwd");
        return VT_OK;
    }
    hipLaunchKernelGGL(k_ln_fwd, dim3(blocks_for(R, NT / 64)), dim3(NT), 0, S(stream), x, R, C, gamma, beta, act, eps,
                       y, xhat, rstd);
    VT_LAUNCH_CHECK("vt_layernorm_fwd");
    return VT_OK;
}

int vt_layernorm_bwd(const float* dy, const float* xhat, const float* rstd, int64_t R, int C, const float* gamma,
                     const float* beta, int act, float* dx, float* dgamma, float* dbeta, int accumulate_params,
                     float* ws, int64_t ws_floats, void* stream) {
    VT_CHECK_ARG(R > 0 && C > 0, "vt_layernorm_bwd: shape");
    hipStream_t st = S(stream);
    if (C <= 256) {
        int64_t blocks = (R + 63) / 64;
        if (blocks > 1024) blocks = 1024;
        if (blocks * 2 * C > ws_floats) blocks = ws_floats / (2 * C);
        VT_CHECK_ARG(blocks >= 1, "vt_layernorm_bwd: workspace too small");
        const int64_t rpb = (R + blocks - 1) / blocks;
        blocks = (R + rpb - 1) / rpb;
        const dim3 grid((unsigned)blocks);
#define VT_LNB(CPL) hipLaunchKernelGGL(k_ln_bwd16<CPL>, grid, dim3(NT), 0, st, dy, xhat, rstd, R, C, gamma, beta, act, \
                                       rpb, dx, ws)
        if (C <= 32) VT_LNB(2);
        else if (C <= 64) VT_LNB(4);
        else if (C <= 128) VT_LNB(8);
        else VT_LNB(16);
#undef VT_LNB
        hipLaunchKernelGGL(k_colred16, dim3((unsigned)((2 * C + CR_C - 1) / CR_C)), dim3(NT), 0, st, ws, (int)blocks,
                           2 * C, dgamma, dbeta, C, accumulate_params);
    } else if (C <= 512) {
        int64_t blocks = (R + 63) / 64;
        if (blocks > 1024) blocks = 1024;
        if (blocks * 2 * C > ws_floats) blocks = ws_floats / (2 * C);
        VT_CHECK_ARG(blocks >= 1, "vt_layernorm_bwd: workspace too small");
        const int64_t rpb = (R + blocks - 1) / blocks;
        blocks = (R + rpb - 1) / rpb;
        hipLaunchKernelGGL(k_ln_bwd<8>, dim3((unsigned)blocks), dim3(NT), 0, st, dy, xhat, rstd, R, C, gamma, beta,
                           act, rpb, dx, ws);
        hipLaunchKernelGGL(k_reduce_parts, dim3(2 * C), dim3(NT), 0, st, ws, (int)blocks, 2 * C, dgamma,
                           dbeta, C, accumulate_params);
    } else {
        VT_CHECK_ARG(ws_floats >= 2 * R * C, "vt_layernorm_bwd: workspace too small (wide)");
        hipLaunchKernelGGL(k_ln_bwd_wide, dim3((unsigned)R), dim3(NT), 0, st, dy, xhat, rstd, C, gamma, beta, act, dx,
                           ws);
        hipLaunchKernelGGL(k_reduce_parts, dim3(2 * C), dim3(NT), 0, st, ws, (int)R, 2 * C, dgamma, dbeta,
                           C, accumulate_params);
// ... 116 lines not shown
    float* db_now = dg_now + C;
    BnFin f = fin_of(2, M);
    f.dgamma = dg_now;
    f.dbeta = db_now;
    f.pg = dgamma;
    f.pb = dbeta;
    f.pacc = accumulate_params;
    col_partial_fin(2, x, dy, M, C, rpb, blocks, mean, rstd, gamma, beta, act, ws, st, f, &dr);
    bn_dx_vec(dy, x, M, C, mean, rstd, gamma, beta, act, dg_now, db_now, dx, st, &dr);
    VT_LAUNCH_CHECK("vt_batchnorm_bwd_dropout");
    return VT_OK;
}

int vt_batchnorm_bwd_coef(const float* dy, const float* x, int64_t M, int C, const float* mean, const float* rstd,
                          const float* gamma, const float* beta, int act, float* dgamma, float* dbeta,
                          int accumulate_params, float* bnp, float* ws, int64_t ws_floats, void* stream) {
    VT_CHECK_ARG(M > 0 && C > 0 && C <= 256 && bnp, "vt_batchnorm_bwd_coef: shape");
    int64_t rpb;
    const int blocks = bn_blocks(M, ws_floats, C, &rpb);
    VT_CHECK_ARG(blocks >= 1, "vt_batchnorm_bwd_coef: workspace too small");
    hipStream_t st = S(stream);
    float* dg_now = bnp + 4 * C;
    float* db_now = bnp + 5 * C;
    BnFin f = fin_of(2, M);
    f.mean = const_cast<float*>(mean);
    f.rstd = const_cast<float*>(rstd);
    f.dgamma = dg_now;
    f.dbeta = db_now;
    f.bnp = bnp;
    f.gamma = gamma;
    f.beta = beta;
    f.pg = dgamma;
    f.pb = dbeta;
    f.pacc = accumulate_params;
    col_partial_fin(2, x, dy, M, C, rpb, blocks, mean, rstd, gamma, beta, act, ws, st, f);
    VT_LAUNCH_CHECK("vt_batchnorm_bwd_coef");
    return VT_OK;
}

int vt_batchnorm_eval(const float* x, int64_t M, int C, const float* run_mean, const float* run_var, float eps,
                      const float* gamma, const float* beta, int act, float* y, void* stream) {
    VT_CHECK_ARG(M > 0 && C > 0, "vt_batchnorm_eval: shape");
    hipLaunchKernelGGL(k_bn_eval, dim3(blocks_for(M * C)), dim3(256), 0, S(stream), x, M, C, run_mean, run_var, eps,
                       gamma, beta, act, y);
    VT_LAUNCH_CHECK("vt_batchnorm_eval");
    return VT_OK;
}

int vt_syncbn_sums(const float* x, const float* dy, int64_t M, int C, int which, const float* mean,
                   const float* rstd, const float* gamma, const float* beta, int act, double* sums, float* ws,
                   int64_t ws_floats, void* stream) {
    VT_CHECK_ARG(M > 0 && C > 0 && C <= 256 && which >= 0 && which <= 2 && sums, "vt_syncbn_sums: shape");
    VT_CHECK_ARG(which == 0 || mean, "vt_syncbn_sums: mean needed");
    VT_CHECK_ARG(which < 2 || (dy && rstd && gamma && beta), "vt_syncbn_sums: backward arguments");
    int64_t rpb;
    const int blocks = bn_blocks(M, ws_floats, C, &rpb);
    VT_CHECK_ARG(blocks >= 1, "vt_syncbn_sums: workspace too small");
    hipStream_t st = S(stream);
    col_partial_vec(which, x, dy, M, C, rpb, blocks, mean, rstd, gamma, beta, act, ws, st, no_fin());
    hipLaunchKernelGGL(k_sbn_sums, dim3(C), dim3(NT), 0, st, ws, blocks, C, M, sums);
    VT_LAUNCH_CHECK("vt_syncbn_sums");
    return VT_OK;
}

int vt_syncbn_stats(const double* sums, int C, int which, float eps, float momentum, float* mean, float* rstd,
                    float* run_mean, float* run_var, float* dgamma, float* dbeta, int accumulate, void* stream) {
    VT_CHECK_ARG(sums && C > 0 && which >= 0 && which <= 2, "vt_syncbn_stats: arguments");
    VT_CHECK_ARG((which == 0 && mean) || (which == 1 && mean && rstd) || (which == 2 && dgamma && dbeta),
                 "vt_syncbn_stats: outputs");
    hipLaunchKernelGGL(k_sbn_stats, dim3(blocks_for(C)), dim3(256), 0, S(stream), sums, C, which, eps, momentum, mean,
                       rstd, run_mean, run_var, dgamma, dbeta, accumulate);
    VT_LAUNCH_CHECK("vt_syncbn_stats");
    return VT_OK;
}

int vt_batchnorm_apply(const float* x, int64_t M, int C, const float* mean, const float* rstd, const float* gamma,
                       const float* beta, int act, float* y, void* stream) {
    VT_CHECK_ARG(M > 0 && C > 0 && C <= BNV_C, "vt_batchnorm_apply: shape");
    bn_apply_vec(x, M, C, mean, rstd, gamma, beta, act, y, S(stream));
    VT_LAUNCH_CHECK("vt_batchnorm_apply");
    return VT_OK;
}

int vt_syncbn_bwd_dx(const float* dy, const float* x, int64_t M, int C, const float* mean, const float* rstd,
                     const float* gamma, const float* beta, int act, const double* sums, float* dx, float* ws,
                     void* stream) {
    VT_CHECK_ARG(M > 0 && C > 0 && C <= BNV_C && sums && ws, "vt_syncbn_bwd_dx: arguments");
    hipStream_t st = S(stream);
    float* dg = ws;
    float* db = ws + C;
    hipLaunchKernelGGL(k_sbn_dsum, dim3(blocks_for(C)), dim3(256), 0, st, sums, C, dg, db);
    const int64_t n = M * C;
#define VT_F(A)                                                                                                   \
    hipLaunchKernelGGL(k_bn_dx4<A>, dim3(bnv_blocks(n)), dim3(NT), 0, st, dy, x, n, (int64_t)1, C, mean, rstd, \
                       gamma, beta, dg, db, dx)
    VT_ACT_SWITCH(act, VT_F)
#undef VT_F
    VT_LAUNCH_CHECK("vt_syncbn_bwd_dx");
    return VT_OK;
}

int vt_act_fwd(const float* x, int64_t n, int act, float* y, void* stream) {
    VT_CHECK_ARG(n > 0, "vt_act_fwd: n");
    hipLaunchKernelGGL(k_act_fwd, dim3(blocks_for(n)), dim3(256), 0, S(stream), x, n, act, y);
    VT_LAUNCH_CHECK("vt_act_fwd");
    return VT_OK;
}

int vt_act_bwd(const float* dy, const float* x, int64_t n, int act, float* dx, void* stream) {
    VT_CHECK_ARG(n > 0, "vt_act_bwd: n");
    hipLaunchKernelGGL(k_act_bwd, dim3(blocks_for(n)), dim3(256), 0, S(stream), dy, x, n, act, dx);
    VT_LAUNCH_CHECK("vt_act_bwd");
    return VT_OK;
}

}
```

### vae-teb_amd/vaeteb/model.py

```python
import math
import os

import torch
import torch.nn as nn

from . import _lib, ops


_PAR = {"on": False, "next": 1}
MAX_SIDE = int(__import__("os").environ.get("VAETEB_MAX_SIDE_STREAMS", "3"))
GRAD_SIDE = int(__import__("os").environ.get("VAETEB_GRAD_SIDE_STREAM", "3"))
HEAD_GRAD_SIDE = int(__import__("os").environ.get("VAETEB_HEAD_GRAD_SIDE_STREAM", "1"))
LSTM_GRAD_SIDE = int(__import__("os").environ.get("VAETEB_LSTM_GRAD_SIDE_STREAM", "0"))
CAPTURE_BRANCHES = __import__("os").environ.get("VAETEB_CAPTURE_BRANCHES", "0") == "1"
PREPASS = int(__import__("os").environ.get("VAETEB_PREPASS", "0"))
PREPASS_SIDE = 3
_SIDE = {}


def side_stream(device, i):
    s = _SIDE.get((device, i))
    if s is None:
        s = _SIDE[(device, i)] = torch.cuda.Stream(device=device)
        ops.SIDE_STREAMS.append(s)
# ... 155 lines not shown
    def _build_fused_spec(self):
        dims, lns, acts, params = [self.input_norm.weight.shape[0]], [], [], [self.input_norm.weight,
                                                                               self.input_norm.bias]
        eps = {self.input_norm.eps}
        for (idx, has_ln, act) in self._plan:
            lin = self.body[idx]
            if lin.mfma:
                return None
            ln = self.body[idx + 1] if has_ln else None
            dims.append(lin.out_features)
            lns.append(has_ln)
            acts.append(act if has_ln else "none")
            params += [lin.weight, lin.bias, ln.weight if ln else None, ln.bias if ln else None]
            if ln is not None:
                eps.add(ln.eps)
        if len(eps) != 1 or not ops.MlpSpec.supported(dims):
            return None
        skip = 0
        if self.use_skip_connection:
            skip = 1 if isinstance(self.skip_proj, nn.Identity) else 2
        params += [self.skip_proj.weight, self.skip_proj.bias] if skip == 2 else [None, None]
        key = (tuple(dims), tuple(lns), tuple(acts), skip)
        if getattr(self, "_spec_key", None) != key:
            self._spec = ops.MlpSpec(dims, lns, acts, skip, eps.pop())
            self._spec_key = key
        return self._spec, params

    def forward(self, x):
        return _drain(self.stages(x))

    def stages(self, x):
        if x.is_cuda and self.fused:
            fs = self._fused_spec()
            if fs is not None:
                return ops.resmlp(x, *fs, bf16=self.bf16)
        x0 = self.input_norm(x)
        h = x0
        for (idx, has_ln, act) in self._plan:
            yield
            lin = self.body[idx]
            if has_ln and not lin.mfma and ops.linear_ln_fused_ok(lin.in_features, lin.out_features):
                ln = self.body[idx + 1]
                h = ops.linear_ln_act(h, lin.weight, lin.bias, ln.weight, ln.bias, act, ln.eps)
                continue
            h = lin(h)
            if has_ln:
                h = self.body[idx + 1](h, act)
        if self.use_skip_connection:
            s = x0 if isinstance(self.skip_proj, nn.Identity) else self.skip_proj(x0)
            h = h + s
        return h


class _ConvWeight(nn.Module):
    def __init__(self, cin, cout, k):
        super().__init__()
        self.in_channels, self.out_channels, self.kernel_size = cin, cout, k
        self.weight = nn.Parameter(torch.empty(cout, cin, k))
        nn.init.xavier_uniform_(self.weight)


class _BatchNorm(nn.Module):
    def __init__(self, c, momentum=0.9, eps=1e-5):
        super().__init__()
        self.momentum, self.eps = momentum, eps
        self.weight = nn.Parameter(torch.ones(c))
        self.bias = nn.Parameter(torch.zeros(c))
        self.register_buffer("running_mean", torch.zeros(c))
        self.register_buffer("running_var", torch.ones(c))
        self.register_buffer("num_batches_tracked", torch.tensor(0, dtype=torch.long))


class ConvBlock(nn.Module):

    def __init__(self, cin, cout, k, causal, up=False, tanh=False):
        super().__init__()
        self.causal, self.up, self.tanh = causal, up, tanh
        self.bf16 = False
        self.conv = _ConvWeight(cin, cout, k)
        self.bn_layer = _BatchNorm(cout)
        self.sync_bn = False
        self.sync_group = None

    def forward(self, x, xin=None, vout=False):
        bn = self.bn_layer
        if xin is not None or vout:
            out = ops.conv_bn_act(x, self.conv.weight, bn.weight, bn.bias, bn.running_mean, bn.running_var,
                                  mode=0 if self.causal else 1, up=self.up, act="tanh" if self.tanh else "relu",
                                  momentum=bn.momentum, eps=bn.eps, bf16=self.bf16, xin=xin, vout=vout)
            if not getattr(bn, "_vt_batched", False):
                bn.num_batches_tracked.add_(1)
            return out
        if not self.training:
            return ops.conv_bn_eval(x, self.conv.weight, bn.weight, bn.bias, bn.running_mean, bn.running_var,
                                    mode=0 if self.causal else 1, up=self.up, act="tanh" if self.tanh else "relu",
                                    eps=bn.eps, bf16=self.bf16)
        if self.sync_bn:
            y = ops.sync_conv_bn_act(x, self.conv.weight, bn.weight, bn.bias, bn.running_mean, bn.running_var,
                                     mode=0 if self.causal else 1, up=self.up, act="tanh" if self.tanh else "relu",
                                     momentum=bn.momentum, eps=bn.eps, bf16=self.bf16, group=self.sync_group)
        else:
            y = ops.conv_bn_act(x, self.conv.weight, bn.weight, bn.bias, bn.running_mean, bn.running_var,
                                mode=0 if self.causal else 1, up=self.up, act="tanh" if self.tanh else "relu",
                                momentum=bn.momentum, eps=bn.eps, bf16=self.bf16)
        if not getattr(bn, "_vt_batched", False):
            bn.num_batches_tracked.add_(1)
        return y


CONV_FOLD = int(os.environ.get("VAETEB_CONV_FOLD", "0"))


class ConvStack(nn.Sequential):

    def forward(self, x):
        blocks = list(self)
        if not (CONV_FOLD and len(blocks) > 1 and x.is_cuda and
                all(isinstance(b, ConvBlock) and b.training and b.bf16 == "bf16" and not b.sync_bn for b in blocks) and
                not any(b.tanh for b in blocks[:-1]) and
                torch.is_grad_enabled() and all(b.conv.weight.requires_grad for b in blocks[:-1])):
            return super().forward(x)
        xin = None
        for i, blk in enumerate(blocks):
            if i == len(blocks) - 1:
                return blk(x, xin=xin)
            x, xin = blk(x, xin=xin, vout=True)


def convert_sync_batchnorm(module, process_group=None):
    for m in module.modules():
        if isinstance(m, ConvBlock):
            m.sync_bn = True
            m.sync_group = process_group
    return module


class LSTM(nn.Module):

    def __init__(self, input_size, hidden_size=64, num_layers=4):
        super().__init__()
        self.input_size, self.hidden_size, self.num_layers = input_size, hidden_size, num_layers
        self.half = False
        for l in range(num_layers):
            din = input_size if l == 0 else hidden_size
            w_ih = nn.Parameter(torch.empty(4 * hidden_size, din))
            w_hh = nn.Parameter(torch.empty(4 * hidden_size, hidden_size))
            nn.init.orthogonal_(w_ih)
            nn.init.orthogonal_(w_hh)
            b_ih = nn.Parameter(torch.zeros(4 * hidden_size))
            b_hh = nn.Parameter(torch.zeros(4 * hidden_size))
            with torch.no_grad():
                b_hh[hidden_size:2 * hidden_size].fill_(1.0)
            setattr(self, f"weight_ih_l{l}", w_ih)
            setattr(self, f"weight_hh_l{l}", w_hh)
            setattr(self, f"bias_ih_l{l}", b_ih)
            setattr(self, f"bias_hh_l{l}", b_hh)

    def flat(self):
        out = []
        for l in range(self.num_layers):
            out += [getattr(self, f"weight_ih_l{l}"), getattr(self, f"weight_hh_l{l}"),
                    getattr(self, f"bias_ih_l{l}"), getattr(self, f"bias_hh_l{l}")]
        return out

    def forward(self, x):
        return ops.lstm(x, self.flat(), half=self.half)


def _seq1(m):
    s = nn.Sequential()
    s.add_module("0", m)
    return s


class SourceEncoder(nn.Module):

    def __init__(self, input_channels=130):
        super().__init__()
        self.mlp = ResidualMLP(input_channels, geometric_schedule(130, 32, 5), final_activation=False)
        self.conv = ConvStack(*[ConvBlock(32, 32, k, causal=True) for k in (3, 5, 7)])
        self.fused_norm = LayerNorm(32)
        self.lstm_norm = LayerNorm(64)
        self.lstm = LSTM(32, 64, 4)
        self.pre_output = ResidualMLP(64, geometric_schedule(64, 32, 4), final_activation=True)
        self.mu_layer = ResidualMLP(32, geometric_schedule(32, 32, 4), final_activation=False)

    def forward(self, x):
        return _drain(self.stages(x))

    def stages(self, x):
        h = self.mlp(x)
        yield
        h = self.conv(h)
        yield
        h = self.lstm(self.fused_norm(h))
        yield
        h = self.pre_output(self.lstm_norm(h))
        yield
        return self.mu_layer(h)
# ... 347 lines not shown
```

### vae-teb_amd/vaeteb/ops.py

```python
import ctypes
import os

import torch

from . import _lib
from ._lib import call, ptr

ACT = {"none": 0, "relu": 1, "gelu": 2, "tanh": 3}


class _Workspace:

    def __init__(self):
        self.buf = {}

    def get(self, nfloats, device, slot=0):
        key = (device.index, slot, _lib.stream() if device.type == "cuda" else 0)
        b = self.buf.get(key)
        if b is None or b.numel() < nfloats:
            b = torch.empty(max(int(nfloats), 1 << 20), dtype=torch.float32, device=device)
            self.buf[key] = b
        return b


# ... 453 lines not shown
                     ptr(xh), ptr(dz16), R, gp, pg.acc, ptr(wsw), wsw.numel(), _st())
        else:
            ws_floats = spec.sizes(R, bool(bf16))[2]
            ws = WS.get(ws_floats, xh.device, 5)
            call("vt_resmlp_bf16_bwd" if bf16 else "vt_resmlp_bwd", spec.L, spec.dims, spec.ln, spec.act, spec.skip,
                 spec.eps, pp, ptr(g2), ptr(xh), ptr(rs), R, ptr(dx), spec.grad_pointers(grads), pg.acc, ptr(ws),
                 ws.numel(), _st())
        res = pg.result()
        out = [None] * len(params)
        for i, gt in zip(present, res):
            out[i] = gt
        return (dx.reshape(ctx.shape), None, None, *out)


def resmlp(x, spec, params, bf16=False):
    return ResMLPF.apply(x, spec, h16_flag(bf16), *params)


class LayerNormActF(torch.autograd.Function):
    @staticmethod
    def forward(ctx, x, g, b, act, eps):
        _check(x, g, b)
        C = x.shape[-1]
        x2 = x.reshape(-1, C).contiguous()
        R = x2.shape[0]
        y = torch.empty_like(x2)
        xhat = torch.empty_like(x2)
        rstd = torch.empty(R, device=x.device)
        call("vt_layernorm_fwd", ptr(x2), R, C, ptr(g), ptr(b), ACT[act], eps, ptr(y), ptr(xhat), ptr(rstd), _st())
        ctx.save_for_backward(xhat, rstd)
        ctx.params = (g, b)
        ctx.act, ctx.shape = act, x.shape
        return y.reshape(x.shape)

    @staticmethod
    def backward(ctx, gy):
        xhat, rstd = ctx.saved_tensors
        g, b = ctx.params
        R, C = xhat.shape
        gy2 = gy.reshape(R, C).contiguous()
        gx = torch.empty_like(xhat)
        pg = _ParamGrads([g, b], [True, True])
        need = 2 * C * max(1024, R if C > 512 else 0)
        ws = WS.get(need, xhat.device, 2)
        call("vt_layernorm_bwd", ptr(gy2), ptr(xhat), ptr(rstd), R, C, ptr(g), ptr(b), ACT[ctx.act], ptr(gx),
             ptr(pg.out[0]), ptr(pg.out[1]), pg.acc, ptr(ws), ws.numel(), _st())
        gg, gbeta = pg.result()
        return gx.reshape(ctx.shape), gg, gbeta, None, None


_CONV_WS = {}
_CONV_SHADOW = {}


def _conv_shadow(w, prepass=False):
    Cout, Cin, K = w.shape
    key = (w.data_ptr(), Cout, Cin, K)
    sh = _CONV_SHADOW.get(key)
    dt = _shadow_dtype()
    if sh is None or sh[0].dtype != dt:
        up32 = lambda n: (n + 31) // 32 * 32
        sh = (torch.empty(Cout * K * up32(Cin), dtype=dt, device=w.device),
              torch.empty(Cin * K * up32(Cout), dtype=dt, device=w.device))
        _CONV_SHADOW[key] = sh
        _FRESH.pop(key, None)
    if prepass or not (_take_prepared(key) or _fresh(key, w)):
        call("vt_conv1d_bf16_shadow", ptr(w), Cout, Cin, K, ptr(sh[0]), ptr(sh[1]), _st())
    return sh


def _conv_bn_ws(*shape):
    n = _CONV_WS.get(shape)
    if n is None:
        import ctypes
        f = ctypes.c_int64()
        call("vt_conv1d_bn_workspace_floats", *shape, ctypes.byref(f))
        n = _CONV_WS[shape] = max(int(f.value), 4096 * shape[3] + 2 * shape[3])
    return n


class ConvBNActF(torch.autograd.Function):

    @staticmethod
    def forward(ctx, x, w, g, b, run_mean, run_var, mode, up, act, momentum, eps, bf16=False, xin=None, vout=False):
        _check(x, w, g, b)
        if (xin is not None or vout) and bf16 != "bf16":
            raise ValueError("the conv-stack BatchNorm fold needs the bf16 conv kernels (no fp32 / fp16 form)")
        _h16(bf16)
        B, L, Cin = x.shape
        Cout, _, K = w.shape
        x = x.contiguous()
        Lo = _lib.lib().fns["vt_conv1d_out_len"](L, K, mode, up)
        conv = torch.empty((B, Lo, Cout), device=x.device)
        y = None if vout else torch.empty_like(conv)
        mean = torch.empty(Cout, device=x.device)
        rstd = torch.empty(Cout, device=x.device)
        ws = WS.get(_conv_bn_ws(B, L, Cin, Cout, K, mode, up), x.device, 2)
        w16t = None
        if bf16:
            w16, w16t = _conv_shadow(w)
            tail = (B, L, Cin, ptr(w16), Cout, K, mode, up, ptr(g), ptr(b), ACT[act], eps, momentum, ptr(conv),
                    None if vout else ptr(y), ptr(mean), ptr(rstd), ptr(run_mean), ptr(run_var), ptr(ws), ws.numel(),
                    _st())
            if xin is not None:
                call("vt_conv1d_bn_fwd_bf16_in", ptr(x), *(ptr(t) for t in xin[:4]), xin[4], *tail)
            else:
                call("vt_conv1d_bn_fwd_bf16", ptr(x), *tail)
        else:
            call("vt_conv1d_bn_fwd", ptr(x), B, L, Cin, ptr(w), Cout, K, mode, up, ptr(g), ptr(b), ACT[act], eps,
                 momentum, ptr(conv), ptr(y), ptr(mean), ptr(rstd), ptr(run_mean), ptr(run_var), ptr(ws), ws.numel(),
                 _st())
        ctx.save_for_backward(x, conv, mean, rstd, w16t, *(xin[:4] if xin is not None else ()))
        ctx.params = (w, g, b)
        ctx.cfg = (mode, up, act, bf16)
        ctx.in_act = None if xin is None else xin[4]
        if vout:
            ctx.mark_non_differentiable(mean, rstd)
            ctx.set_materialize_grads(False)
            return conv, mean, rstd
        return y

    @staticmethod
    def backward(ctx, gy, *_):
        x, conv, mean, rstd, w16t, *xin = ctx.saved_tensors
        if gy is None:
            gy = torch.zeros_like(conv)
        w, g, b = ctx.params
        mode, up, act, bf16 = ctx.cfg
        _h16(bf16)
        inb = (*(ptr(t) for t in xin), ctx.in_act) if xin else None
        B, L, Cin = x.shape
        Cout, _, K = w.shape
        Lo = conv.shape[1]
        gy = gy.contiguous()
        pbn = _ParamGrads([g, b], [True, True])
        ws = WS.get(4096 * Cout + 2 * Cout, x.device, 2)
        M = B * Lo
        fused = bf16 and ctx.needs_input_grad[0]
        pad = K - 1 if mode == 0 else (K - 1) // 2
        bwd16 = fused and CONV_BWD16 and K <= 11 and B <= 65535 and Cout <= 1024 and \
            (mode == 1 and L * (2 if up else 1) > pad or mode == 0 and not up)
        if bwd16:
            bnp = torch.empty(6 * Cout, device=x.device)
            call("vt_batchnorm_bwd_coef", ptr(gy), ptr(conv), M, Cout, ptr(mean), ptr(rstd), ptr(g), ptr(b),
                 ACT[act], ptr(pbn.out[0]), ptr(pbn.out[1]), pbn.acc, ptr(bnp), ptr(ws), ws.numel(), _st())
            c32 = (Cout + 31) // 32 * 32
            dxbn = torch.empty(M * c32, dtype=_shadow_dtype(), device=x.device)
            call("vt_batchnorm_bwd_x16", ptr(gy), ptr(conv), ptr(bnp), ACT[act], M, Cout, ptr(dxbn), _st())
            srcs = (dxbn,)
            dw_args = lambda wsx: (ptr(dxbn), c32, ptr(x), B, L, Cin, Cout, K, mode, up, ptr(pw.out[0]), pw.acc,
                                   ptr(wsx), wsx.numel(), _st())
            fn = "vt_conv1d_bwd_weight_bf16_dy16s"
            if inb:
                dw_args = lambda wsx: (None, ptr(dxbn), c32, ptr(x), *inb, B, L, Cin, Cout, K, mode, up,
                                       ptr(pw.out[0]), pw.acc, ptr(wsx), wsx.numel(), _st())
                fn = "vt_conv1d_bwd_weight_bf16_in"
        elif fused:
            bnp = torch.empty(6 * Cout, device=x.device)
            call("vt_batchnorm_bwd_coef", ptr(gy), ptr(conv), M, Cout, ptr(mean), ptr(rstd), ptr(g), ptr(b),
                 ACT[act], ptr(pbn.out[0]), ptr(pbn.out[1]), pbn.acc, ptr(bnp), ptr(ws), ws.numel(), _st())
            dxbn = torch.empty(M * ((Cout + 7) // 8 * 8), dtype=torch.bfloat16, device=x.device)
            srcs = (dxbn,)
            dw_args = lambda wsx: (ptr(dxbn), ptr(x), B, L, Cin, Cout, K, mode, up, ptr(pw.out[0]), pw.acc,
                                   ptr(wsx), wsx.numel(), _st())
            fn = "vt_conv1d_bwd_weight_bf16_dy16"
            if inb:
                dw_args = lambda wsx: (None, ptr(dxbn), (Cout + 7) // 8 * 8, ptr(x), *inb, B, L, Cin, Cout, K, mode,
                                       up, ptr(pw.out[0]), pw.acc, ptr(wsx), wsx.numel(), _st())
                fn = "vt_conv1d_bwd_weight_bf16_in"
        else:
            gconv = torch.empty_like(conv)
            call("vt_batchnorm_bwd", ptr(gy), ptr(conv), M, Cout, ptr(mean), ptr(rstd), ptr(g), ptr(b), ACT[act],
                 ptr(gconv), ptr(pbn.out[0]), ptr(pbn.out[1]), pbn.acc, ptr(ws), ws.numel(), _st())
            srcs = (gconv,)
            dw_args = lambda wsx: (ptr(gconv), ptr(x), B, L, Cin, Cout, K, mode, up, ptr(pw.out[0]), pw.acc,
                                   ptr(wsx), wsx.numel(), _st())
            fn = "vt_conv1d_bwd_weight_bf16" if bf16 else "vt_conv1d_direct_bwd_weight"
            if inb:
                raise RuntimeError("conv-stack fold: the block input's gradient is required")
        gx = None
        if ctx.needs_input_grad[0]:
            gx = torch.empty_like(x)
            if bwd16:
                edge = WS.get(max(B * 2 * pad * Cin, 1), x.device, 3)
                call("vt_conv1d_bwd_dx16", ptr(dxbn), B, L, Cin, ptr(w16t), Cout, K, mode, up, ptr(gx), ptr(edge),
                     _st())
            elif fused and CONV_DIRECT_DX and not up and (mode == 0 or L > pad):
                edge = WS.get(max(B * 2 * pad * Cin, 1), x.device, 3)
                call("vt_conv1d_bwd_dx_bf16_bn", ptr(gy), ptr(conv), ptr(bnp), ACT[act], M, B, L, Cin, ptr(w16t),
                     Cout, K, mode, up, ptr(gx), ptr(edge), ptr(dxbn), _st())
            else:
                gpad = WS.get(B * (Lo + K - 1) * Cin, x.device, 3)
                if fused:
                    call("vt_conv1d_bwd_gpad_bf16_bn", ptr(gy), ptr(conv), ptr(bnp), ACT[act], M, B, L, Cin,
                         ptr(w16t), Cout, K, mode, up, ptr(gpad), ptr(dxbn), _st())
                else:
                    call("vt_conv1d_direct_bwd_gpad", ptr(gconv), B, L, Cin, ptr(w), Cout, K, mode, up, ptr(gpad),
                         _st())
                call("vt_conv1d_fold", ptr(gpad), B, L, Cin, Cout, K, mode, up, ptr(gx), 0, _st())
        pw = _ParamGrads([w], [ctx.needs_input_grad[1]])
        if pw.out[0] is not None:
            side = GRAD_STREAM if (pw.direct and GRAD_STREAM is not None) else None
            if side is not None and side.cuda_stream != _lib.stream():
                _lib.wait_for(side)
                with torch.cuda.stream(side):
                    ws1 = WS.get(WS_LINEAR, x.device, 1)
                    call(fn, *dw_args(ws1))
                for t in (*srcs, x, *xin):
                    t.record_stream(side)
            else:
                ws1 = WS.get(WS_LINEAR, x.device, 1)
                call(fn, *dw_args(ws1))
        gw, = pw.result()
        gg, gb = pbn.result()
        return gx, gw, gg, gb, None, None, None, None, None, None, None, None, None, None


class SyncConvBNActF(torch.autograd.Function):

    @staticmethod
    def forward(ctx, x, w, g, b, run_mean, run_var, mode, up, act, momentum, eps, bf16, group):
        import torch.distributed as dist
        if x.is_cuda and torch.cuda.is_current_stream_capturing():
            raise RuntimeError("SyncBatchNorm conv blocks cannot be captured into a hipGraph "
                               "(cross-rank statistics need a collective inside the step); train them eagerly")
        _check(x, w, g, b)
        B, L, Cin = x.shape
        Cout, _, K = w.shape
        x = x.contiguous()
        Lo = _lib.lib().fns["vt_conv1d_out_len"](L, K, mode, up)
        conv = torch.empty((B, Lo, Cout), device=x.device)
        if bf16:
            _h16(bf16)
            w16, w16t = _conv_shadow(w)
            call("vt_conv1d_fwd_bf16", ptr(x), B, L, Cin, ptr(w16), Cout, K, mode, up, ptr(conv), _st())
        else:
            w16t = None
            call("vt_conv1d_direct_fwd", ptr(x), B, L, Cin, ptr(w), Cout, K, mode, up, ptr(conv), _st())
        M = B * Lo
        mean = torch.empty(Cout, device=x.device)
        rstd = torch.empty(Cout, device=x.device)
        sums = torch.empty(2 * Cout + 1, dtype=torch.float64, device=x.device)
        ws = WS.get(4096 * Cout * 2 + 2 * Cout, x.device, 2)
        for which, outs in ((0, (ptr(mean), None, None, None)), (1, (ptr(mean), ptr(rstd), ptr(run_mean),
                                                                     ptr(run_var)))):
            call("vt_syncbn_sums", ptr(conv), None, M, Cout, which, ptr(mean), None, None, None, 0, ptr(sums),
                 ptr(ws), ws.numel(), _st())
            dist.all_reduce(sums, op=dist.ReduceOp.SUM, group=group)
            call("vt_syncbn_stats", ptr(sums), Cout, which, eps, momentum, *outs, None, None, 0, _st())
        y = torch.empty_like(conv)
        call("vt_batchnorm_apply", ptr(conv), M, Cout, ptr(mean), ptr(rstd), ptr(g), ptr(b), ACT[act], ptr(y), _st())
        ctx.save_for_backward(x, conv, mean, rstd, w16t)
        ctx.params = (w, g, b)
        ctx.cfg = (mode, up, act, bf16, group)
        return y

    @staticmethod
    def backward(ctx, gy):
        import torch.distributed as dist
        x, conv, mean, rstd, w16t = ctx.saved_tensors
        w, g, b = ctx.params
        mode, up, act, bf16, group = ctx.cfg
        _h16(bf16)
        B, L, Cin = x.shape
        Cout, _, K = w.shape
        Lo = conv.shape[1]
        M = B * Lo
        gy = gy.contiguous()
        pbn = _ParamGrads([g, b], [True, True])
        sums = torch.empty(2 * Cout + 1, dtype=torch.float64, device=x.device)
        ws = WS.get(4096 * Cout * 2 + 2 * Cout, x.device, 2)
        call("vt_syncbn_sums", ptr(conv), ptr(gy), M, Cout, 2, ptr(mean), ptr(rstd), ptr(g), ptr(b), ACT[act],
             ptr(sums), ptr(ws), ws.numel(), _st())
        call("vt_syncbn_stats", ptr(sums), Cout, 2, 0.0, 0.0, None, None, None, None, ptr(pbn.out[0]),
             ptr(pbn.out[1]), pbn.acc, _st())
        dist.all_reduce(sums, op=dist.ReduceOp.SUM, group=group)
        gconv = torch.empty_like(conv)
        call("vt_syncbn_bwd_dx", ptr(gy), ptr(conv), M, Cout, ptr(mean), ptr(rstd), ptr(g), ptr(b), ACT[act],
             ptr(sums), ptr(gconv), ptr(ws), _st())
        gx = None
        if ctx.needs_input_grad[0]:
            gx = torch.empty_like(x)
            gpad = WS.get(B * (Lo + K - 1) * Cin, x.device, 3)
            if bf16:
                call("vt_conv1d_bwd_gpad_bf16", ptr(gconv), B, L, Cin, ptr(w16t), Cout, K, mode, up, ptr(gpad), _st())
            else:
                call("vt_conv1d_direct_bwd_gpad", ptr(gconv), B, L, Cin, ptr(w), Cout, K, mode, up, ptr(gpad), _st())
            call("vt_conv1d_fold", ptr(gpad), B, L, Cin, Cout, K, mode, up, ptr(gx), 0, _st())
        pw = _ParamGrads([w], [ctx.needs_input_grad[1]])
        if pw.out[0] is not None:
            ws1 = WS.get(WS_LINEAR, x.device, 1)
            fn = "vt_conv1d_bwd_weight_bf16" if bf16 else "vt_conv1d_direct_bwd_weight"
            call(fn, ptr(gconv), ptr(x), B, L, Cin, Cout, K, mode, up, ptr(pw.out[0]), pw.acc, ptr(ws1), ws1.numel(),
                 _st())
        gw, = pw.result()
        gg, gb = pbn.result()
        return gx, gw, gg, gb, None, None, None, None, None, None, None, None, None, None, None

# ... 328 lines not shown
    @staticmethod
    def backward(ctx, gnll, gmse):
        g_mu, g_lv, g_lin = ctx.saved_tensors
        for t, s in ((g_mu, gnll), (g_lv, gnll), (g_lin, gmse)):
            if t.numel() and s is not None:
                call("vt_scale_by_device_scalar", ptr(t), t.numel(), ptr(s.reshape(1).contiguous()), _st())
        return g_mu, g_lv, None, (g_lin if ctx.has_lin else None), None, None


class CatLastF(torch.autograd.Function):

    @staticmethod
    def forward(ctx, *xs):
        xs = [x.contiguous() for x in xs]
        widths = [int(x.shape[-1]) for x in xs]
        W, lead = sum(widths), tuple(xs[0].shape[:-1])
        R = xs[0].numel() // widths[0]
        out = torch.empty(*lead, W, device=xs[0].device, dtype=torch.float32)
        c0 = 0
        for x, w in zip(xs, widths):
            call("vt_copy_cols", ptr(x), R, w, 0, w, ptr(out), W, c0, _st())
            c0 += w
        ctx.widths, ctx.lead, ctx.R = widths, lead, R
        return out

    @staticmethod
    def backward(ctx, g):
        g = g.contiguous()
        W = sum(ctx.widths)
        outs, c0 = [], 0
        for w, need in zip(ctx.widths, ctx.needs_input_grad):
            d = None
            if need:
                d = torch.empty(*ctx.lead, w, device=g.device, dtype=torch.float32)
                call("vt_copy_cols", ptr(g), ctx.R, W, c0, w, ptr(d), w, 0, _st())
            outs.append(d)
            c0 += w
        return tuple(outs)


class ClampF(torch.autograd.Function):

    @staticmethod
    def forward(ctx, x, lo, hi):
        ctx.save_for_backward(x)
        ctx.lo, ctx.hi = float(lo), float(hi)
        return torch.clamp(x, lo, hi)

    @staticmethod
    def backward(ctx, g):
        (x,) = ctx.saved_tensors
        g = g.contiguous()
        gx = torch.empty_like(x)
        call("vt_clamp_bwd", ptr(g), ptr(x), x.numel(), ctx.lo, ctx.hi, ptr(gx), _st())
        return gx, None, None


def clamp(x, lo, hi):
    if x.is_cuda and x.dtype == torch.float32 and x.is_contiguous() and x.numel() > 0 and x.requires_grad:
        return ClampF.apply(x, lo, hi)
    return torch.clamp(x, lo, hi)


def cat_last(xs):
    if len(xs) > 1 and all(x.is_cuda and x.dtype == torch.float32 and x.shape[:-1] == xs[0].shape[:-1]
                           and x.numel() > 0 for x in xs):
        return CatLastF.apply(*xs)
    return torch.cat(xs, dim=-1)


def linear(x, w, b=None, mfma=False):
    return LinearF.apply(x, w, b, mfma)


def linear_ln_act(x, w, b, g, beta, act="none", eps=1e-5):
    return LinearLNActF.apply(x, w, b, g, beta, act, eps)


def layer_norm_act(x, g, b, act="none", eps=1e-5):
    return LayerNormActF.apply(x, g, b, act, eps)


def conv_bn_act(x, w, g, b, run_mean, run_var, mode, up=False, act="relu", momentum=0.9, eps=1e-5, bf16=False,
                xin=None, vout=False):
    out = ConvBNActF.apply(x, w, g, b, run_mean, run_var, int(mode), int(up), act, momentum, eps, h16_flag(bf16), xin,
                           bool(vout))
    if not vout:
        return out
    conv, mean, rstd = out
    return conv, (mean, rstd, g, b, ACT[act])


def lstm(x, params, half=False):
    return LSTMF.apply(x, bool(half), *params)


def latent(mu_c, lv_q, mu_y, lv_p, eps):
    return LatentF.apply(mu_c, lv_q, mu_y, lv_p, eps)


def output_losses(mu, lv, y, lin=None, y_st=None, y_ph=None):
    return OutputLossF.apply(mu, lv, y, lin, y_st, y_ph)
```

Baseline: 33880.

## Hand off conv-stack activations as staged 16-bit rows between blocks

Inside a training conv stack, each block's BatchNorm+activation output is written directly as padded bf16/f16 rows, already upsampled when the next block upsamples. The next block's forward conv and its weight-gradient kernel read these rows instead of the fp32 activation, and the fp32 output tensor is dropped. This aims to cut fp32 activation write/read traffic and the per-load upsampling and BN work. It adds new kernel variants and stricter alignment and shape requirements. The input activation is now kept at 16-bit precision for the weight gradient.

```diff
diff --git a/include/vaeteb.h b/include/vaeteb.h
--- a/include/vaeteb.h
+++ b/include/vaeteb.h
@@ -259,6 +259,15 @@
                                  const float* in_rstd, const float* in_gamma, const float* in_beta, int in_act, int B,
                                  int L_in, int Cin, int Cout, int K, int mode, int up, float* dW, int accumulate,
                                  float* ws, int64_t ws_floats, void* stream);
+int vt_batchnorm_apply_x16(const float* x, int B, int L, int C, const float* mean, const float* rstd,
+                           const float* gamma, const float* beta, int act, int up, void* y16, void* stream);
+int vt_conv1d_bn_fwd_bf16_x16(const float* X, const void* X16, int B, int L_in, int Cin, const void* w16, int Cout,
+                              int K, int mode, int up, const float* gamma, const float* beta, int act, float eps,
+                              float momentum, float* conv_out, float* Y, float* mean, float* rstd, float* run_mean,
+                              float* run_var, float* ws, int64_t ws_floats, void* Y16, int y16_up, void* stream);
+int vt_conv1d_bwd_weight_bf16_x16(const void* dY16, int dys, const void* X16, int B, int L_in, int Cin, int Cout,
+                                  int K, int mode, int up, float* dW, int accumulate, float* ws, int64_t ws_floats,
+                                  void* stream);
 int vt_batchnorm_bwd_x16(const float* dY, const float* Xc, const float* bnp, int act, int64_t M, int C, void* d16,
                          void* stream);
 int vt_conv1d_bwd_dx16(const void* d16, int B, int L_in, int Cin, const void* w16t, int Cout, int K, int mode, int up,
diff --git a/vae-teb_amd/csrc/conv.h b/vae-teb_amd/csrc/conv.h
--- a/vae-teb_amd/csrc/conv.h
+++ b/vae-teb_amd/csrc/conv.h
@@ -1,6 +1,7 @@
 #pragma once
 #include "bnbwd.h"
 #include "common.h"
+#include "x16.h"
 
 namespace vt {
 
@@ -43,6 +44,14 @@
 }
 
 
+__device__ __forceinline__ void up_rows(int t, int L_in, int& i0, int& i1, float& l1) {
+    float s = (t + 0.5f) * 0.5f - 0.5f;
+    s = s < 0.f ? 0.f : s;
+    i0 = (int)s;
+    i1 = i0 + 1 < L_in ? i0 + 1 : L_in - 1;
+    l1 = s - (float)i0;
+}
+
 __device__ __forceinline__ bool src_row(const Geo& g, int tp, int& i0, int& i1, float& l1) {
     int t = tp - g.pad;
     if (g.mode == 0) {
@@ -58,11 +67,7 @@
         l1 = 0.f;
         return true;
     }
-    float s = (t + 0.5f) * 0.5f - 0.5f;
-    s = s < 0.f ? 0.f : s;
-    i0 = (int)s;
-    i1 = i0 + 1 < g.L_in ? i0 + 1 : g.L_in - 1;
-    l1 = s - (float)i0;
+    up_rows(t, g.L_in, i0, i1, l1);
     return true;
 }
 
@@ -155,6 +160,12 @@
                       int pK = 0, int pCo = 0, int pCi = 0);
 int cfw16_launch(const float* x, const Geo& g, const void* w16, float* y, int Lo, float* stats, hipStream_t st,
                  const BnIn* ibn = nullptr);
+static inline Geo x16_geo(int B, int L_in, int Cin, int Cout, int K, int mode, int up) {
+    return geo(B, L_in * (up ? 2 : 1), Cin, Cout, K, mode, 0);
+}
+int cfw16_x16_launch(const void* x16, const Geo& g, const void* w16, float* y, int Lo, float* stats, hipStream_t st);
+int bn_apply_x16_launch(const float* x, int B, int L, int C, const float* mean, const float* rstd,
+                        const float* gamma, const float* beta, int act, int up, void* out16, hipStream_t st);
 void fold_edges_launch(float* dx, const float* edge, int B, int L, int pad, int C, hipStream_t st);
 int bn_apply_launch(const float* x, int64_t M, int C, const float* mean, const float* rstd, const float* gamma,
                     const float* beta, int act, float* y, hipStream_t st);
diff --git a/vae-teb_amd/csrc/conv_bf16.hip b/vae-teb_amd/csrc/conv_bf16.hip
--- a/vae-teb_amd/csrc/conv_bf16.hip
+++ b/vae-teb_amd/csrc/conv_bf16.hip
@@ -575,7 +575,8 @@
 static int bn_fwd_bf16(const float* X, int B, int L_in, int Cin, const void* w16, int Cout, int K, int mode, int up,
                        const float* gamma, const float* beta, int act, float eps, float momentum, float* conv_out,
                        float* Y, float* mean, float* rstd, float* run_mean, float* run_var, float* ws,
-                       int64_t ws_floats, hipStream_t st, const BnIn* ibn, const char* who) {
+                       int64_t ws_floats, hipStream_t st, const BnIn* ibn, const char* who,
+                       const void* X16 = nullptr, void* Y16 = nullptr, int y16_up = 0) {
     VT_CHECK_ARG(B > 0 && L_in > 0 && Cin > 0 && Cout > 0 && K > 0 && K <= KMAXB && (mode == 0 || mode == 1),
                  "%s: shape (K <= %d)", who, KMAXB);
     Geo g = geo(B, L_in, Cin, Cout, K, mode, up);
@@ -583,11 +584,27 @@
     const int TP = bf_launch(nullptr, g, nullptr, cin32, nullptr, g.L_out, nullptr, nullptr);
     const int tps = cdiv(g.L_out, TP);
     VT_CHECK_ARG(ws && ws_floats >= (int64_t)B * tps * 2 * Cout, "%s: workspace too small", who);
-    if (bf_launch(X, g, w16, cin32, conv_out, g.L_out, ws, st, nullptr, FoldOut{-1, 0, nullptr}, ibn) < 0) return VT_ERR_ARG;
+    if (X16) {
+        const int tp = cfw16_x16_launch(X16, x16_geo(B, L_in, Cin, Cout, K, mode, up), w16, conv_out, g.L_out, ws, st);
+        VT_CHECK_ARG(tp == TP, "%s: staged input rows (16-byte aligned, the window of %d channels in LDS)", who, Cin);
+    } else if (bf_launch(X, g, w16, cin32, conv_out, g.L_out, ws, st, nullptr, FoldOut{-1, 0, nullptr}, ibn) < 0)
+        return VT_ERR_ARG;
     bn_stats_finalize_launch(ws, tps, B, TP, g.L_out, Cout, eps, momentum, mean, rstd, run_mean, run_var, st);
     if (Y) bn_apply_launch(conv_out, (int64_t)B * g.L_out, Cout, mean, rstd, gamma, beta, act, Y, st);
+    if (Y16 && bn_apply_x16_launch(conv_out, B, g.L_out, Cout, mean, rstd, gamma, beta, act, y16_up, Y16, st))
+        return VT_ERR_ARG;
     VT_LAUNCH_CHECK(who);
     return VT_OK;
+}
+
+int vt_conv1d_bn_fwd_bf16_x16(const float* X, const void* X16, int B, int L_in, int Cin, const void* w16, int Cout,
+                              int K, int mode, int up, const float* gamma, const float* beta, int act, float eps,
+                              float momentum, float* conv_out, float* Y, float* mean, float* rstd, float* run_mean,
+                              float* run_var, float* ws, int64_t ws_floats, void* Y16, int y16_up, void* stream) {
+    VT_CHECK_ARG((X != nullptr) != (X16 != nullptr), "vt_conv1d_bn_fwd_bf16_x16: exactly one of X, X16");
+    return bn_fwd_bf16(X, B, L_in, Cin, w16, Cout, K, mode, up, gamma, beta, act, eps, momentum, conv_out, Y, mean,
+                       rstd, run_mean, run_var, ws, ws_floats, S(stream), nullptr, "vt_conv1d_bn_fwd_bf16_x16", X16,
+                       Y16, y16_up);
 }
 
 int vt_conv1d_bn_fwd_bf16(const float* X, int B, int L_in, int Cin, const void* w16, int Cout, int K, int mode,
diff --git a/vae-teb_amd/csrc/conv_dw16.hip b/vae-teb_amd/csrc/conv_dw16.hip
--- a/vae-teb_amd/csrc/conv_dw16.hip
+++ b/vae-teb_amd/csrc/conv_dw16.hip
@@ -169,14 +169,17 @@
 constexpr int CDW_UF = 8;
 constexpr int CDW_UF_WIDE = 12;
 
-template <int K, int PPW, int NWV, int CR = DWR, bool IBN = false, typename H = __bf16>
+template <int K, int PPW, int NWV, int CR = DWR, bool IBN = false, typename H = __bf16, bool X16 = false>
 __global__ __launch_bounds__(64 * NWV) void k_cdw16(const H* __restrict__ dyb16, int dys,
                                                    const float* __restrict__ x, Geo g, int64_t rows_per_split,
                                                    int NTc, int npairs, int dstride, int xstride,
-                                                   float* __restrict__ part, int64_t total, BnIn bi, int ipo) {
+                                                   float* __restrict__ part, int64_t total, BnIn bi, int ipo,
+                                                   const H* __restrict__ xh, int xcs) {
+    static_assert(!(X16 && IBN), "k_cdw16: staged rows already carry the previous block's BatchNorm");
     constexpr int NT = 64 * NWV;
     constexpr int UD = CR == DWR ? CDW_UD * 256 / NT : CR * 4 / NT;
-    constexpr int UF = CR == DWR ? CDW_UF * 256 / NT : CDW_UF_WIDE * 256 / NT;
+    constexpr int UF = X16 ? 1 : (CR == DWR ? CDW_UF * 256 / NT : CDW_UF_WIDE * 256 / NT);
+    constexpr int UX = X16 ? cdw16_x16_ux(CR, K, NT) : 1;
     extern __shared__ __attribute__((aligned(16))) char lb_raw[];
     H* const lb = reinterpret_cast<H*>(lb_raw);
     H* ds = lb;
@@ -206,6 +209,8 @@
     if constexpr (IBN) stage_bn_in(bi, g.Cin, ip, cin16);
     hv8<H> dv[UD];
     float4 fv[UF];
+    hv8<H> xv[UX];
+    const int osegs = cin16 / 8;
     struct Chunk {
         int b, t0, n, lo, hi, off, nv;
     };
@@ -225,6 +230,25 @@
 #pragma unroll
                 for (int j = 0; j < 8; ++j) dv[u][j] = (H)0.f;
             }
+        }
+        if constexpr (X16) {
+            const H* xb = xh + (int64_t)c.b * g.L_in * xcs;
+#pragma unroll
+            for (int u = 0; u < UX; ++u) {
+                const int i = tid + NT * u;
+                const int t = i / osegs, o = i - t * osegs;
+                int i0 = 0, i1 = 0;
+                float l1 = 0.f;
+                const bool in = i < (CR + K - 1) * osegs && t < c.n + K - 1 && 8 * o < xcs &&
+                                src_row(g, c.t0 + t, i0, i1, l1);
+                xv[u] = *(const hv8<H>*)(xb + (int64_t)(in ? i0 : 0) * xcs + (in ? 8 * o : 0));
+                if (!in) {
+#pragma unroll
+                    for (int j = 0; j < 8; ++j) xv[u][j] = (H)0.f;
+                }
+            }
+            c.lo = c.hi = c.off = c.nv = 0;
+            return;
         }
         src_span(g, c.t0, c.n + K - 1, c.lo, c.hi);
         const int64_t f0 = ((int64_t)c.b * g.L_in + c.lo) * g.Cin;
@@ -258,6 +282,16 @@
                 *(hv8<H>*)(ds + t * dstride + 8 * sg) = dv[u];
             }
         }
+        if constexpr (X16) {
+#pragma unroll
+            for (int u = 0; u < UX; ++u) {
+                const int i = tid + NT * u;
+                if (i < (CR + K - 1) * osegs) {
+                    const int t = i / osegs, o = i - t * osegs;
+                    *(hv8<H>*)(xs + t * xstride + 8 * o) = xv[u];
+                }
+            }
+        } else {
 #pragma unroll
         for (int u = 0; u < UF; ++u)
             if (tid + NT * u < cur.nv) reinterpret_cast<float4*>(F)[tid + NT * u] = fv[u];
@@ -287,6 +321,7 @@
                 *(hv8<H>*)(xs + t * xstride + cb) = v;
             }
         }
+        }
         __syncthreads();
         const int64_t rn = r + cur.n;
         Chunk nxt = cur;
@@ -335,10 +370,10 @@
 
 static int bwd_weight(const float* dY, const float* X, int B, int L_in, int Cin, int Cout, int K, int mode, int up,
                       float* dW, int accumulate, float* ws, int64_t ws_floats, hipStream_t st, const void* dy16,
-                      int dys = 0, const BnIn* ibn = nullptr) {
+                      int dys = 0, const BnIn* ibn = nullptr, const void* x16 = nullptr) {
     VT_CHECK_ARG(B > 0 && L_in > 0 && K > 0 && K <= KMAXB && Cin > 0 && Cout > 0 && Cin <= 128 && Cout <= 128,
                  "vt_conv1d_bwd_weight_bf16: shape (K <= %d, channels <= 128)", KMAXB);
-    Geo g = geo(B, L_in, Cin, Cout, K, mode, up);
+    Geo g = x16 ? x16_geo(B, L_in, Cin, Cout, K, mode, up) : geo(B, L_in, Cin, Cout, K, mode, up);
     const int NTc = cdiv(Cin, 16), npairs = cdiv(Cout, 16) * NTc;
     const int ppw_max = K <= 3 ? 6 : (K <= 5 ? 4 : (K <= 7 ? 3 : 2));
     const int ppw = cdiv(npairs, 4) < ppw_max ? cdiv(npairs, 4) : ppw_max;
@@ -376,19 +411,42 @@
     const BnIn bi = ibn ? *ibn : BnIn{};
     const int ib = ibn ? 16 * (16 * cdiv(Cin, 16)) : 0;
     const int ipo_w = ((int)lds_wide + 15) & ~15, ipo_f = ((int)lds_flat + 15) & ~15, ipo_d = ((int)lds + 15) & ~15;
+    const bool xwide = x16 && (g_conv_kern & 8) && cdiv(Cout, 16) <= 2 && cdw16_x16_fits(256, K, Cin) && rps >= 256;
+    const int xcs = x16_stride(Cin);
+    const size_t lds_xw = (size_t)cdw16_x16_lds(256, dstride, xstride), lds_x = (size_t)cdw16_x16_lds(DWR, dstride, xstride);
+    if (x16)
+        VT_CHECK_ARG(!ibn && dy16 && ((uintptr_t)x16 & 15) == 0 && ((uintptr_t)dy16 & 15) == 0 && dys % 8 == 0 &&
+                         cdw16_x16_fits(DWR, K, Cin) && (int64_t)(xwide ? lds_xw : lds_x) <= X16_LDS_MAX,
+                     "vt_conv1d_bwd_weight_bf16_x16: 16-byte aligned 16-bit dY16 / X16 rows required");
+#define VT_DWB_X16(HT, NW, CRR, LDSX)                                                                           \
+    hipLaunchKernelGGL((k_cdw16<KK, PP, NW, CRR, false, HT, true>), grid, dim3(64 * NW), LDSX, st,              \
+                       (const HT*)dy16, dys, nullptr, g, rps, NTc, npairs, dstride, xstride, ws, 0, BnIn{}, 0,  \
+                       (const HT*)x16, xcs)
 #define VT_DWB_ONE(IB, HT)                                                                                      \
-    if (wide && nwv == 8)                                                                                       \
+    if (xwide && nwv == 8)                                                                                      \
+        VT_DWB_X16(HT, 8, 256, lds_xw);                                                                         \
+    else if (xwide)                                                                                             \
+        VT_DWB_X16(HT, 4, 256, lds_xw);                                                                         \
+    else if (x16 && nwv == 8)                                                                                   \
+        VT_DWB_X16(HT, 8, DWR, lds_x);                                                                          \
+    else if (x16)                                                                                               \
+        VT_DWB_X16(HT, 4, DWR, lds_x);                                                                          \
+    else if (wide && nwv == 8)                                                                                  \
         hipLaunchKernelGGL((k_cdw16<KK, PP, 8, 256, IB, HT>), grid, dim3(512), ipo_w + ib, st, (const HT*)dy16,   \
-                           dys, X, g, rps, NTc, npairs, dstride, xstride, ws, total_x, bi, ipo_w);             \
+                           dys, X, g, rps, NTc, npairs, dstride, xstride, ws, total_x, bi, ipo_w,                  \
+                           (const HT*)nullptr, 0);                                                                 \
     else if (wide)                                                                                              \
         hipLaunchKernelGGL((k_cdw16<KK, PP, 4, 256, IB, HT>), grid, dim3(256), ipo_w + ib, st, (const HT*)dy16,   \
-                           dys, X, g, rps, NTc, npairs, dstride, xstride, ws, total_x, bi, ipo_w);             \
+                           dys, X, g, rps, NTc, npairs, dstride, xstride, ws, total_x, bi, ipo_w,                  \
+                           (const HT*)nullptr, 0);                                                                 \
     else if (flat && nwv == 8)                                                                                  \
         hipLaunchKernelGGL((k_cdw16<KK, PP, 8, DWR, IB, HT>), grid, dim3(512), ipo_f + ib, st, (const HT*)dy16,   \
-                           dys, X, g, rps, NTc, npairs, dstride, xstride, ws, total_x, bi, ipo_f);             \
+                           dys, X, g, rps, NTc, npairs, dstride, xstride, ws, total_x, bi, ipo_f,                  \
+                           (const HT*)nullptr, 0);                                                                 \
     else if (flat)                                                                                              \
         hipLaunchKernelGGL((k_cdw16<KK, PP, 4, DWR, IB, HT>), grid, dim3(256), ipo_f + ib, st, (const HT*)dy16,   \
-                           dys, X, g, rps, NTc, npairs, dstride, xstride, ws, total_x, bi, ipo_f);             \
+                           dys, X, g, rps, NTc, npairs, dstride, xstride, ws, total_x, bi, ipo_f,                  \
+                           (const HT*)nullptr, 0);                                                                 \
     else if (dy16 && nwv == 8)                                                                                  \
         hipLaunchKernelGGL((k_conv_dw_bf16<KK, PP, true, 8, IB, HT>), grid, dim3(512), ipo_d + ib, st, dY, X, g,  \
                            rps, NTc, npairs, dstride, xstride, ws, (const HT*)dy16, dys, bi, ipo_d);           \
@@ -423,6 +481,7 @@
 #undef VT_DWB2
 #undef VT_DWB
 #undef VT_DWB_ONE
+#undef VT_DWB_X16
     const int rc = sum_splits_launch(ws, (int)splits, nout, dW, accumulate, st);
     if (rc) return rc;
     VT_LAUNCH_CHECK("vt_conv1d_bwd_weight_bf16");
@@ -448,6 +507,15 @@
                  "vt_conv1d_bwd_weight_bf16_dy16s: null dY16 or row stride %d (a multiple of 8 >= ceil8(Cout))", dys);
     return bwd_weight(nullptr, X, B, L_in, Cin, Cout, K, mode, up, dW, accumulate, ws, ws_floats, S(stream),
                       dY16, dys);
+}
+
+int vt_conv1d_bwd_weight_bf16_x16(const void* dY16, int dys, const void* X16, int B, int L_in, int Cin, int Cout,
+                                  int K, int mode, int up, float* dW, int accumulate, float* ws, int64_t ws_floats,
+                                  void* stream) {
+    VT_CHECK_ARG(dY16 != nullptr && X16 != nullptr && dys >= ((Cout + 7) & ~7) && dys % 8 == 0,
+                 "vt_conv1d_bwd_weight_bf16_x16: null dY16 / X16 or row stride %d (a multiple of 8 >= ceil8(Cout))", dys);
+    return bwd_weight(nullptr, nullptr, B, L_in, Cin, Cout, K, mode, up, dW, accumulate, ws, ws_floats, S(stream),
+                      dY16, dys, nullptr, X16);
 }
 
 int vt_conv1d_bwd_weight_bf16_in(const float* dY, const void* dY16, int dys, const float* X, const float* in_mean,
diff --git a/vae-teb_amd/csrc/conv_fwd16.hip b/vae-teb_amd/csrc/conv_fwd16.hip
--- a/vae-teb_amd/csrc/conv_fwd16.hip
+++ b/vae-teb_amd/csrc/conv_fwd16.hip
@@ -16,10 +16,12 @@
     static constexpr int WBYTES = K * TC * RS * 2;
 };
 
-template <int K, int NT, bool IBN = false, typename H = __bf16>
+template <int K, int NT, bool IBN = false, typename H = __bf16, bool X16 = false>
 __global__ __launch_bounds__(256) void k_cfw16(const float* __restrict__ x, Geo g, int nch,
                                                const H* __restrict__ w16, float* __restrict__ y, int Lo,
-                                               float* __restrict__ stats, int64_t total, BnIn bi, int ipo) {
+                                               float* __restrict__ stats, int64_t total, BnIn bi, int ipo,
+                                               const H* __restrict__ xh, int xcs) {
+    static_assert(!(X16 && IBN), "k_cfw16: staged rows already carry the previous block's BatchNorm");
     using C = FCfg<K, NT>;
     constexpr int PM = C::PM, TC = C::TC, TP = C::TP, WIN = C::WIN;
     extern __shared__ __attribute__((aligned(16))) char lb_raw[];
@@ -45,6 +47,33 @@
     load_taps(0);
     float* ip = reinterpret_cast<float*>(reinterpret_cast<char*>(lb) + ipo);
     if constexpr (IBN) stage_bn_in(bi, g.Cin, ip, cin32);
+    if constexpr (X16) {
+        const int segs = 4 * nch, xsegs = xcs >> 3;
+        const H* xb = xh + (int64_t)b * g.L_in * xcs;
+        constexpr int U = 4;
+        for (int j0 = tid; j0 < WIN * segs; j0 += 256 * U) {
+            hv8<H> v[U];
+#pragma unroll
+            for (int u = 0; u < U; ++u) {
+                const int i = j0 + 256 * u;
+                const int r = i / segs, s = i - r * segs;
+                int i0 = 0, i1 = 0;
+                float l1 = 0.f;
+                const bool in = i < WIN * segs && t0 + r < Lo + K - 1 && s < xsegs && src_row(g, t0 + r, i0, i1, l1);
+                v[u] = *(const hv8<H>*)(xb + (int64_t)(in ? i0 : 0) * xcs + (in ? 8 * s : 0));
+                if (!in) {
+#pragma unroll
+                    for (int j = 0; j < 8; ++j) v[u][j] = (H)0.f;
+                }
+            }
+#pragma unroll
+            for (int u = 0; u < U; ++u) {
+                const int i = j0 + 256 * u;
+                const int r = i / segs, s = i - r * segs;
+                if (i < WIN * segs) *(hv8<H>*)(xs + ((s >> 2) * WIN + r) * RS + 8 * (s & 3)) = v[u];
+            }
+        }
+    } else {
     int lo, hi;
     src_span(g, t0, WIN < Lo + K - 1 - t0 ? WIN : Lo + K - 1 - t0, lo, hi);
     const int64_t f0 = ((int64_t)b * g.L_in + lo) * g.Cin;
@@ -103,6 +132,7 @@
         }
     }
     __syncthreads();
+    }
     auto store_taps = [&]() {
 #pragma unroll
         for (int it = 0; it < C::NWI; ++it) {
@@ -212,9 +242,22 @@
 
 template <int K, int NT>
 int cfw_nt(const float* x, const Geo& g, const void* w16, float* y, int Lo, float* stats, hipStream_t st,
-           const BnIn* ibn) {
+           const BnIn* ibn, const void* x16) {
     using C = FCfg<K, NT>;
     const int nch = cdiv(g.Cin, 32);
+    if (x16) {
+        const int64_t lds = cfw16_x16_lds(K, NT, nch);
+        if (ibn || g.up || lds > X16_LDS_MAX || ((uintptr_t)x16 & 15)) return VT_ERR_ARG;
+        dim3 grid(cdiv(Lo, C::TP), cdiv(g.Cout, C::TC), g.B);
+        const int xcs = x16_stride(g.Cin);
+        if (h16_format())
+            hipLaunchKernelGGL((k_cfw16<K, NT, false, _Float16, true>), grid, dim3(256), (size_t)lds, st, nullptr, g, nch,
+                               (const _Float16*)w16, y, Lo, stats, 0, BnIn{}, 0, (const _Float16*)x16, xcs);
+        else
+            hipLaunchKernelGGL((k_cfw16<K, NT, false, __bf16, true>), grid, dim3(256), (size_t)lds, st, nullptr, g, nch,
+                               (const __bf16*)w16, y, Lo, stats, 0, BnIn{}, 0, (const __bf16*)x16, xcs);
+        return C::TP;
+    }
     const int src_rows = g.up ? C::WIN / 2 + 3 : C::WIN;
     const int fbytes = (src_rows * g.Cin + 8) * 4;
     const int rest = fbytes > C::WBYTES ? fbytes : C::WBYTES;
@@ -229,26 +272,43 @@
     if (h16_format()) {
         if (ibn) return VT_ERR_ARG;
         hipLaunchKernelGGL((k_cfw16<K, NT, false, _Float16>), grid, dim3(256), lds, st, x, g, nch,
-                           (const _Float16*)w16, y, Lo, stats, total, bi, ipo);
+                           (const _Float16*)w16, y, Lo, stats, total, bi, ipo, nullptr, 0);
     } else if (ibn)
         hipLaunchKernelGGL((k_cfw16<K, NT, true, __bf16>), grid, dim3(256), lds, st, x, g, nch, (const __bf16*)w16, y, Lo, stats,
-                           total, bi, ipo);
+                           total, bi, ipo, nullptr, 0);
     else
         hipLaunchKernelGGL((k_cfw16<K, NT, false, __bf16>), grid, dim3(256), lds, st, x, g, nch, (const __bf16*)w16, y, Lo, stats,
-                           total, bi, ipo);
+                           total, bi, ipo, nullptr, 0);
     return C::TP;
 }
 
 template <int K>
 int cfw_k(const float* x, const Geo& g, const void* w16, float* y, int Lo, float* stats, hipStream_t st,
-          const BnIn* ibn) {
+          const BnIn* ibn, const void* x16) {
     switch (cdiv(g.Cout, 16) < 6 ? cdiv(g.Cout, 16) : 6) {
-        case 1: return cfw_nt<K, 1>(x, g, w16, y, Lo, stats, st, ibn);
-        case 2: return cfw_nt<K, 2>(x, g, w16, y, Lo, stats, st, ibn);
-        case 3: return cfw_nt<K, 3>(x, g, w16, y, Lo, stats, st, ibn);
-        case 4: return cfw_nt<K, 4>(x, g, w16, y, Lo, stats, st, ibn);
-        case 5: return cfw_nt<K, 5>(x, g, w16, y, Lo, stats, st, ibn);
-        default: return cfw_nt<K, 6>(x, g, w16, y, Lo, stats, st, ibn);
+        case 1: return cfw_nt<K, 1>(x, g, w16, y, Lo, stats, st, ibn, x16);
+        case 2: return cfw_nt<K, 2>(x, g, w16, y, Lo, stats, st, ibn, x16);
+        case 3: return cfw_nt<K, 3>(x, g, w16, y, Lo, stats, st, ibn, x16);
+        case 4: return cfw_nt<K, 4>(x, g, w16, y, Lo, stats, st, ibn, x16);
+        case 5: return cfw_nt<K, 5>(x, g, w16, y, Lo, stats, st, ibn, x16);
+        default: return cfw_nt<K, 6>(x, g, w16, y, Lo, stats, st, ibn, x16);
+    }
+}
+
+int cfw16_any(const float* x, const Geo& g, const void* w16, float* y, int Lo, float* stats, hipStream_t st,
+              const BnIn* ibn, const void* x16) {
+    switch (g.K) {
+        case 1: return cfw_k<1>(x, g, w16, y, Lo, stats, st, ibn, x16);
+        case 2: return cfw_k<2>(x, g, w16, y, Lo, stats, st, ibn, x16);
+        case 3: return cfw_k<3>(x, g, w16, y, Lo, stats, st, ibn, x16);
+        case 4: return cfw_k<4>(x, g, w16, y, Lo, stats, st, ibn, x16);
+        case 5: return cfw_k<5>(x, g, w16, y, Lo, stats, st, ibn, x16);
+        case 6: return cfw_k<6>(x, g, w16, y, Lo, stats, st, ibn, x16);
+        case 7: return cfw_k<7>(x, g, w16, y, Lo, stats, st, ibn, x16);
+        case 8: return cfw_k<8>(x, g, w16, y, Lo, stats, st, ibn, x16);
+        case 9: return cfw_k<9>(x, g, w16, y, Lo, stats, st, ibn, x16);
+        case 10: return cfw_k<10>(x, g, w16, y, Lo, stats, st, ibn, x16);
+        default: return cfw_k<11>(x, g, w16, y, Lo, stats, st, ibn, x16);
     }
 }
 
@@ -256,19 +316,11 @@
 
 int cfw16_launch(const float* x, const Geo& g, const void* w16, float* y, int Lo, float* stats, hipStream_t st,
                  const BnIn* ibn) {
-    switch (g.K) {
-        case 1: return cfw_k<1>(x, g, w16, y, Lo, stats, st, ibn);
-        case 2: return cfw_k<2>(x, g, w16, y, Lo, stats, st, ibn);
-        case 3: return cfw_k<3>(x, g, w16, y, Lo, stats, st, ibn);
-        case 4: return cfw_k<4>(x, g, w16, y, Lo, stats, st, ibn);
-        case 5: return cfw_k<5>(x, g, w16, y, Lo, stats, st, ibn);
-        case 6: return cfw_k<6>(x, g, w16, y, Lo, stats, st, ibn);
-        case 7: return cfw_k<7>(x, g, w16, y, Lo, stats, st, ibn);
-        case 8: return cfw_k<8>(x, g, w16, y, Lo, stats, st, ibn);
-        case 9: return cfw_k<9>(x, g, w16, y, Lo, stats, st, ibn);
-        case 10: return cfw_k<10>(x, g, w16, y, Lo, stats, st, ibn);
-        default: return cfw_k<11>(x, g, w16, y, Lo, stats, st, ibn);
-    }
-}
-
-}
+    return cfw16_any(x, g, w16, y, Lo, stats, st, ibn, nullptr);
+}
+
+int cfw16_x16_launch(const void* x16, const Geo& g, const void* w16, float* y, int Lo, float* stats, hipStream_t st) {
+    return x16 ? cfw16_any(nullptr, g, w16, y, Lo, stats, st, nullptr, x16) : VT_ERR_ARG;
+}
+
+}
diff --git a/vae-teb_amd/csrc/norm.hip b/vae-teb_amd/csrc/norm.hip
--- a/vae-teb_amd/csrc/norm.hip
+++ b/vae-teb_amd/csrc/norm.hip
@@ -2,7 +2,9 @@
 
 #include "bnbwd.h"
 #include "common.h"
+#include "conv.h"
 #include "dropout.h"
+#include "h16.h"
 
 namespace vt {
 
@@ -577,6 +579,95 @@
                 y[j + e] = bn_fwd_val(x[j + e], q.x, q.y, q.z, q.w, ACT);
             }
         }
+    }
+}
+
+template <typename H, int ACT, bool UP>
+__global__ __launch_bounds__(NT) void k_bn_apply_x16(const float* __restrict__ x, int L, int C,
+                                                     const float* __restrict__ mean, const float* __restrict__ rstd,
+                                                     const float* __restrict__ gamma, const float* __restrict__ beta,
+                                                     H* __restrict__ out, int cs, int64_t total) {
+    constexpr int TR = x16_apply_rows(UP);
+    extern __shared__ __attribute__((aligned(16))) float4 xl[];
+    float4* p = xl;
+    H* img = reinterpret_cast<H*>(xl + C);
+    float* yf = reinterpret_cast<float*>(img + X16_APPLY_OUT * cs);
+    const int tid = threadIdx.x, b = blockIdx.y, m0 = blockIdx.x * TR;
+    for (int c = tid; c < C; c += NT) p[c] = make_float4(mean[c], rstd[c], gamma[c], beta[c]);
+    __syncthreads();
+    const int nrow = L - m0 < TR + (UP ? 1 : 0) ? L - m0 : TR + (UP ? 1 : 0);
+    const int n = nrow * C;
+    const int64_t f0 = ((int64_t)b * L + m0) * C, fa = f0 & ~(int64_t)3;
+    const int off = (int)(f0 - fa), nv = (off + n + 3) >> 2;
+    {
+        const int e0 = 4 * tid - off + 4 * C;
+        int r = e0 / C - 4, c = e0 % C;
+        const int rstep = (4 * NT) / C, cstep = (4 * NT) % C;
+        for (int i = tid; i < nv; i += NT) {
+            const int64_t g = fa + 4 * (int64_t)i;
+            float v[4];
+            if (g + 3 < total) {
+                const float4 f = *reinterpret_cast<const float4*>(x + g);
+                v[0] = f.x; v[1] = f.y; v[2] = f.z; v[3] = f.w;
+            } else {
+#pragma unroll
+                for (int j = 0; j < 4; ++j) v[j] = g + j < total ? x[g + j] : 0.f;
+            }
+            int rr = r, cc = c;
+#pragma unroll
+            for (int j = 0; j < 4; ++j) {
+                const int e = 4 * i + j - off;
+                if (e >= 0 && e < n) {
+                    const float4 w = p[cc];
+                    const float y = bn_fwd_val(v[j], w.x, w.y, w.z, w.w, ACT);
+                    if constexpr (UP)
+                        yf[e] = y;
+                    else
+                        img[rr * cs + cc] = (H)y;
+                }
+                if (++cc == C) {
+                    cc = 0;
+                    ++rr;
+                }
+            }
+            r += rstep;
+            c += cstep;
+            if (c >= C) {
+                c -= C;
+                ++r;
+            }
+        }
+    }
+    __syncthreads();
+    const int Lx = UP ? 2 * L : L;
+    const int t_lo = UP ? (m0 == 0 ? 0 : 2 * m0 + 1) : m0;
+    const int t_end = UP ? (2 * (m0 + TR) + 1 < Lx ? 2 * (m0 + TR) + 1 : Lx) : (m0 + TR < L ? m0 + TR : L);
+    const int nt = t_end - t_lo;
+    if constexpr (UP) {
+        int r = tid / C, c = tid % C;
+        const int rstep = NT / C, cstep = NT % C;
+        for (int i = tid; i < nt * C; i += NT) {
+            int i0, i1;
+            float l1;
+            up_rows(t_lo + r, L, i0, i1, l1);
+            img[r * cs + c] = (H)up_lerp(yf[(i0 - m0) * C + c], yf[(i1 - m0) * C + c], l1);
+            r += rstep;
+            c += cstep;
+            if (c >= C) {
+                c -= C;
+                ++r;
+            }
+        }
+        __syncthreads();
+    }
+    const int segs = cs >> 3;
+    for (int i = tid; i < nt * segs; i += NT) {
+        const int r = i / segs, sg = i - r * segs;
+        hv8<H> v = *reinterpret_cast<const hv8<H>*>(img + r * cs + 8 * sg);
+#pragma unroll
+        for (int j = 0; j < 8; ++j)
+            if (8 * sg + j >= C) v[j] = (H)0.f;
+        *reinterpret_cast<hv8<H>*>(out + ((int64_t)b * Lx + t_lo + r) * cs + 8 * sg) = v;
     }
 }
 
@@ -980,6 +1071,27 @@
     else
         hipLaunchKernelGGL(k_bn_apply, dim3(blocks_for(M * C)), dim3(256), 0, st, x, M, C, mean, rstd, gamma, beta,
                            act, y);
+    return VT_OK;
+}
+
+int bn_apply_x16_launch(const float* x, int B, int L, int C, const float* mean, const float* rstd,
+                        const float* gamma, const float* beta, int act, int up, void* out16, hipStream_t st) {
+    if (!x16_apply_ok(B, L, C) || ((uintptr_t)out16 & 15) || ((uintptr_t)x & 15)) {
+        set_error("staged 16-bit rows: shape (B %d <= 65535, L %d, C %d <= %d) or a misaligned pointer", B, L, C,
+                  X16_CMAX);
+        return VT_ERR_ARG;
+    }
+    const int cs = x16_stride(C);
+    const dim3 grid((unsigned)((L + x16_apply_rows(up) - 1) / x16_apply_rows(up)), (unsigned)B);
+    const size_t lds = (size_t)x16_apply_lds(C, up);
+    const int64_t total = (int64_t)B * L * C;
+#define VT_F(A)                                                                                                   \
+    VT_H16(if (up) hipLaunchKernelGGL((k_bn_apply_x16<H, A, true>), grid, dim3(NT), lds, st, x, L, C, mean, rstd,  \
+                                      gamma, beta, (H*)out16, cs, total);                                        \
+           else hipLaunchKernelGGL((k_bn_apply_x16<H, A, false>), grid, dim3(NT), lds, st, x, L, C, mean, rstd,    \
+                                   gamma, beta, (H*)out16, cs, total))
+    VT_ACT_SWITCH(act, VT_F)
+#undef VT_F
     return VT_OK;
 }
 
@@ -1262,6 +1374,14 @@
     return VT_OK;
 }
 
+int vt_batchnorm_apply_x16(const float* x, int B, int L, int C, const float* mean, const float* rstd,
+                           const float* gamma, const float* beta, int act, int up, void* y16, void* stream) {
+    VT_CHECK_ARG(x && mean && rstd && gamma && beta && y16, "vt_batchnorm_apply_x16: null argument");
+    if (bn_apply_x16_launch(x, B, L, C, mean, rstd, gamma, beta, act, up, y16, S(stream))) return VT_ERR_ARG;
+    VT_LAUNCH_CHECK("vt_batchnorm_apply_x16");
+    return VT_OK;
+}
+
 int vt_syncbn_bwd_dx(const float* dy, const float* x, int64_t M, int C, const float* mean, const float* rstd,
                      const float* gamma, const float* beta, int act, const double* sums, float* dx, float* ws,
                      void* stream) {
diff --git a/vae-teb_amd/csrc/x16.h b/vae-teb_amd/csrc/x16.h
--- /dev/null
+++ b/vae-teb_amd/csrc/x16.h
@@ -0,0 +1,35 @@
+#pragma once
+#include <stdint.h>
+
+namespace vt {
+
+constexpr int X16_LDS_MAX = 160 * 1024;
+constexpr int X16_RS = 40;
+constexpr int X16_KMAX = 11;
+
+constexpr int x16_stride(int C) { return (C + 7) & ~7; }
+
+constexpr int X16_CMAX = 128;
+constexpr int X16_APPLY_OUT = 65;
+constexpr int x16_apply_rows(int up) { return up ? 32 : 64; }
+constexpr int64_t x16_apply_lds(int C, int up) {
+    return 16 * (int64_t)C + X16_APPLY_OUT * (int64_t)x16_stride(C) * 2 + (up ? (int64_t)(x16_apply_rows(1) + 1) * C * 4 : 0);
+}
+constexpr bool x16_apply_ok(int B, int L, int C) {
+    return B > 0 && B <= 65535 && L > 0 && L <= (1 << 29) && C > 0 && C <= X16_CMAX;
+}
+
+constexpr int64_t cfw16_x16_lds(int K, int NT, int nch) {
+    const int PM = NT <= 2 ? 4 : 2, TC = 16 * NT, WIN = 64 * PM + K - 1;
+    const int64_t lds = (int64_t)nch * WIN * X16_RS * 2 + (int64_t)K * TC * X16_RS * 2;
+    return lds < 8 * TC * 4 ? 8 * TC * 4 : lds;
+}
+
+constexpr int cdw16_x16_maxseg(int CR) { return CR == 64 ? 16 : 6; }
+constexpr int cdw16_x16_ux(int CR, int K, int nt) { return ((CR + K - 1) * cdw16_x16_maxseg(CR) + nt - 1) / nt; }
+constexpr bool cdw16_x16_fits(int CR, int K, int Cin) { return (Cin + 15) / 16 * 2 <= cdw16_x16_maxseg(CR); }
+constexpr int64_t cdw16_x16_lds(int CR, int dstride, int xstride) {
+    return ((int64_t)CR * dstride + (int64_t)(CR + X16_KMAX + 8) * xstride) * 2;
+}
+
+}
diff --git a/vae-teb_amd/vaeteb/model.py b/vae-teb_amd/vaeteb/model.py
--- a/vae-teb_amd/vaeteb/model.py
+++ b/vae-teb_amd/vaeteb/model.py
@@ -261,12 +261,13 @@
         self.sync_bn = False
         self.sync_group = None
 
-    def forward(self, x, xin=None, vout=False):
+    def forward(self, x, xin=None, vout=False, x16=None, y16=None):
         bn = self.bn_layer
-        if xin is not None or vout:
+        if xin is not None or vout or x16 is not None or y16 is not None:
             out = ops.conv_bn_act(x, self.conv.weight, bn.weight, bn.bias, bn.running_mean, bn.running_var,
                                   mode=0 if self.causal else 1, up=self.up, act="tanh" if self.tanh else "relu",
-                                  momentum=bn.momentum, eps=bn.eps, bf16=self.bf16, xin=xin, vout=vout)
+                                  momentum=bn.momentum, eps=bn.eps, bf16=self.bf16, xin=xin, vout=vout,
+                                  x16=x16, y16=y16)
             if not getattr(bn, "_vt_batched", False):
                 bn.num_batches_tracked.add_(1)
             return out
@@ -292,8 +293,21 @@
 
 class ConvStack(nn.Sequential):
 
+    def _staged(self, blocks, x):
+        return (len(blocks) > 1 and x.is_cuda and
+                all(isinstance(b, ConvBlock) and b.training and b.bf16 and not b.sync_bn for b in blocks) and
+                len({b.bf16 for b in blocks}) == 1 and
+                torch.is_grad_enabled() and all(b.conv.weight.requires_grad for b in blocks[:-1]) and
+                all(b.conv.kernel_size <= 11 and b.conv.in_channels <= 128 and b.conv.out_channels <= 128
+                    for b in blocks[1:]))
+
     def forward(self, x):
         blocks = list(self)
+        if not CONV_FOLD and self._staged(blocks, x):
+            h, rows = blocks[0](x, y16=blocks[1].up)
+            for i in range(1, len(blocks) - 1):
+                h, rows = blocks[i](h, x16=rows, y16=blocks[i + 1].up)
+            return blocks[-1](h, x16=rows)
         if not (CONV_FOLD and len(blocks) > 1 and x.is_cuda and
                 all(isinstance(b, ConvBlock) and b.training and b.bf16 == "bf16" and not b.sync_bn for b in blocks) and
                 not any(b.tanh for b in blocks[:-1]) and
diff --git a/vae-teb_amd/vaeteb/ops.py b/vae-teb_amd/vaeteb/ops.py
--- a/vae-teb_amd/vaeteb/ops.py
+++ b/vae-teb_amd/vaeteb/ops.py
@@ -559,27 +559,41 @@
 class ConvBNActF(torch.autograd.Function):
 
     @staticmethod
-    def forward(ctx, x, w, g, b, run_mean, run_var, mode, up, act, momentum, eps, bf16=False, xin=None, vout=False):
+    def forward(ctx, x, w, g, b, run_mean, run_var, mode, up, act, momentum, eps, bf16=False, xin=None, vout=False,
+                x16=None, y16=None):
         _check(x, w, g, b)
         if (xin is not None or vout) and bf16 != "bf16":
             raise ValueError("the conv-stack BatchNorm fold needs the bf16 conv kernels (no fp32 / fp16 form)")
+        if (x16 is not None or y16 is not None) and (not bf16 or xin is not None or vout):
+            raise ValueError("the staged 16-bit hand-off needs the 16-bit conv kernels (and excludes the fold)")
         _h16(bf16)
         B, L, Cin = x.shape
         Cout, _, K = w.shape
-        x = x.contiguous()
+        if x16 is None:
+            x = x.contiguous()
         Lo = _lib.lib().fns["vt_conv1d_out_len"](L, K, mode, up)
         conv = torch.empty((B, Lo, Cout), device=x.device)
-        y = None if vout else torch.empty_like(conv)
+        y = None if vout or y16 is not None else torch.empty_like(conv)
         mean = torch.empty(Cout, device=x.device)
         rstd = torch.empty(Cout, device=x.device)
         ws = WS.get(_conv_bn_ws(B, L, Cin, Cout, K, mode, up), x.device, 2)
         w16t = None
+        rows = None
         if bf16:
             w16, w16t = _conv_shadow(w)
             tail = (B, L, Cin, ptr(w16), Cout, K, mode, up, ptr(g), ptr(b), ACT[act], eps, momentum, ptr(conv),
-                    None if vout else ptr(y), ptr(mean), ptr(rstd), ptr(run_mean), ptr(run_var), ptr(ws), ws.numel(),
-                    _st())
-            if xin is not None:
+                    None if y is None else ptr(y), ptr(mean), ptr(rstd), ptr(run_mean), ptr(run_var), ptr(ws),
+                    ws.numel(), _st())
+            if x16 is not None or y16 is not None:
+                if y16 is not None:
+                    rows = torch.empty((B, Lo * (2 if y16 else 1), (Cout + 7) // 8 * 8), dtype=_shadow_dtype(),
+                                       device=x.device)
+                if x16 is not None and (x16.dtype != _shadow_dtype() or not x16.is_contiguous() or
+                                        x16.shape != (B, L * (2 if up else 1), (Cin + 7) // 8 * 8)):
+                    raise ValueError(f"staged input rows: {x16.dtype} {tuple(x16.shape)}")
+                call("vt_conv1d_bn_fwd_bf16_x16", None if x16 is not None else ptr(x), ptr(x16), *tail[:-1],
+                     ptr(rows), int(bool(y16)), _st())
+            elif xin is not None:
                 call("vt_conv1d_bn_fwd_bf16_in", ptr(x), *(ptr(t) for t in xin[:4]), xin[4], *tail)
             else:
                 call("vt_conv1d_bn_fwd_bf16", ptr(x), *tail)
@@ -587,14 +601,20 @@
             call("vt_conv1d_bn_fwd", ptr(x), B, L, Cin, ptr(w), Cout, K, mode, up, ptr(g), ptr(b), ACT[act], eps,
                  momentum, ptr(conv), ptr(y), ptr(mean), ptr(rstd), ptr(run_mean), ptr(run_var), ptr(ws), ws.numel(),
                  _st())
-        ctx.save_for_backward(x, conv, mean, rstd, w16t, *(xin[:4] if xin is not None else ()))
+        ctx.save_for_backward(x16 if x16 is not None else x, conv, mean, rstd, w16t,
+                              *(xin[:4] if xin is not None else ()))
         ctx.params = (w, g, b)
         ctx.cfg = (mode, up, act, bf16)
         ctx.in_act = None if xin is None else xin[4]
+        ctx.x16 = (B, L, Cin) if x16 is not None else None
         if vout:
             ctx.mark_non_differentiable(mean, rstd)
             ctx.set_materialize_grads(False)
             return conv, mean, rstd
+        if y16 is not None:
+            ctx.mark_non_differentiable(rows)
+            ctx.set_materialize_grads(False)
+            return torch.empty(1, device=x.device).expand(B, Lo, Cout), rows
         return y
 
     @staticmethod
@@ -606,7 +626,8 @@
         mode, up, act, bf16 = ctx.cfg
         _h16(bf16)
         inb = (*(ptr(t) for t in xin), ctx.in_act) if xin else None
-        B, L, Cin = x.shape
+        x16 = ctx.x16 is not None
+        B, L, Cin = ctx.x16 if x16 else x.shape
         Cout, _, K = w.shape
         Lo = conv.shape[1]
         gy = gy.contiguous()
@@ -632,6 +653,7 @@
                 dw_args = lambda wsx: (None, ptr(dxbn), c32, ptr(x), *inb, B, L, Cin, Cout, K, mode, up,
                                        ptr(pw.out[0]), pw.acc, ptr(wsx), wsx.numel(), _st())
                 fn = "vt_conv1d_bwd_weight_bf16_in"
+            dys = c32
         elif fused:
             bnp = torch.empty(6 * Cout, device=x.device)
             call("vt_batchnorm_bwd_coef", ptr(gy), ptr(conv), M, Cout, ptr(mean), ptr(rstd), ptr(g), ptr(b),
@@ -645,7 +667,10 @@
                 dw_args = lambda wsx: (None, ptr(dxbn), (Cout + 7) // 8 * 8, ptr(x), *inb, B, L, Cin, Cout, K, mode,
                                        up, ptr(pw.out[0]), pw.acc, ptr(wsx), wsx.numel(), _st())
                 fn = "vt_conv1d_bwd_weight_bf16_in"
+            dys = (Cout + 7) // 8 * 8
         else:
+            if x16:
+                raise RuntimeError("staged 16-bit hand-off: the block input's gradient is required")
             gconv = torch.empty_like(conv)
             call("vt_batchnorm_bwd", ptr(gy), ptr(conv), M, Cout, ptr(mean), ptr(rstd), ptr(g), ptr(b), ACT[act],
                  ptr(gconv), ptr(pbn.out[0]), ptr(pbn.out[1]), pbn.acc, ptr(ws), ws.numel(), _st())
@@ -655,9 +680,13 @@
             fn = "vt_conv1d_bwd_weight_bf16" if bf16 else "vt_conv1d_direct_bwd_weight"
             if inb:
                 raise RuntimeError("conv-stack fold: the block input's gradient is required")
+        if x16:
+            dw_args = lambda wsx: (ptr(dxbn), dys, ptr(x), B, L, Cin, Cout, K, mode, up, ptr(pw.out[0]), pw.acc,
+                                   ptr(wsx), wsx.numel(), _st())
+            fn = "vt_conv1d_bwd_weight_bf16_x16"
         gx = None
         if ctx.needs_input_grad[0]:
-            gx = torch.empty_like(x)
+            gx = torch.empty((B, L, Cin), device=conv.device)
             if bwd16:
                 edge = WS.get(max(B * 2 * pad * Cin, 1), x.device, 3)
                 call("vt_conv1d_bwd_dx16", ptr(dxbn), B, L, Cin, ptr(w16t), Cout, K, mode, up, ptr(gx), ptr(edge),
@@ -690,7 +719,7 @@
                 call(fn, *dw_args(ws1))
         gw, = pw.result()
         gg, gb = pbn.result()
-        return gx, gw, gg, gb, None, None, None, None, None, None, None, None, None, None
+        return gx, gw, gg, gb, None, None, None, None, None, None, None, None, None, None, None, None
 
 
 class SyncConvBNActF(torch.autograd.Function):
@@ -1185,9 +1214,9 @@
 
 
 def conv_bn_act(x, w, g, b, run_mean, run_var, mode, up=False, act="relu", momentum=0.9, eps=1e-5, bf16=False,
-                xin=None, vout=False):
+                xin=None, vout=False, x16=None, y16=None):
     out = ConvBNActF.apply(x, w, g, b, run_mean, run_var, int(mode), int(up), act, momentum, eps, h16_flag(bf16), xin,
-                           bool(vout))
+                           bool(vout), x16, None if y16 is None else int(bool(y16)))
     if not vout:
         return out
     conv, mean, rstd = out
```

Result: faster. 34790, median of 6 (+2.7%).
